# gradslam/gradslam

Measured on AMD Instinct MI355X. Metric: frames/sec PointFusion 640x480 RGB-D, higher is better.
Workload: dtype f32

## Files before the change

### gradslam_amd/csrc/build.py

```python
import os
import subprocess
import sys
from concurrent.futures import ThreadPoolExecutor

HERE = os.path.dirname(os.path.abspath(__file__))
SOURCES = ["gs_frame.hip", "gs_assoc.hip", "gs_fuse.hip", "gs_knn.hip", "gs_icp.hip", "gs_icp_loop.hip", "gs_icp_bwd.hip", "gs_ingest.hip", "gs_render.hip", "gs_prune.hip", "gs_bilateral.hip"]
HEADERS = ["gs_common.h", "gs_env.h", "gs_compact.h", "gs_assoc_dev.h", "gs_knn.h", "gs_knn_bbox.h", "gs_icp_math.h", "gs_icp_persist.h", "gs_icp_timeline.h", os.path.join("..", "..", "include", "gradslam_hip.h")]
LIB = os.path.join(HERE, "libgradslam_hip.so")
FLAGS = ["--offload-arch=gfx950", "-O3", "-std=c++17", "-fPIC", "-ffp-contract=off", "-fno-fast-math", "-fno-slp-vectorize",
         "-fvisibility=hidden", "-Wall", "-Wno-unused-function"]


FLAGS += os.environ.get("GRADSLAM_HIP_BUILD_FLAGS", "").split()


def _hipcc():
    for c in (os.environ.get("HIPCC"), "/opt/rocm/bin/hipcc", "hipcc"):
        if c and (os.path.sep not in c or os.path.exists(c)):
            return c
    raise RuntimeError("hipcc not found")


def _stale(target, deps):
    if not os.path.exists(target):
        return True
    t = os.path.getmtime(target)
    return any(os.path.getmtime(d) > t for d in deps)


def build(force=False, verbose=False):
    hipcc = _hipcc()
    stamp = os.path.join(HERE, ".build_flags")
    flags_now = " ".join(FLAGS)
    if not os.path.exists(stamp) or open(stamp).read() != flags_now:
        force = True
    hdrs = [os.path.join(HERE, h) for h in HEADERS]
    jobs = []
    for s in SOURCES:
        src = os.path.join(HERE, s)
        obj = os.path.join(HERE, s.replace(".hip", ".o"))
        if force or _stale(obj, [src] + hdrs):
            jobs.append([hipcc] + FLAGS + ["-c", src, "-o", obj])

    def run(cmd):
        if verbose:
            print(" ".join(cmd))
        r = subprocess.run(cmd, capture_output=True, text=True)
        if r.returncode != 0:
            raise RuntimeError("hipcc failed:\n%s\n%s" % (" ".join(cmd), r.stderr))
        return r.stderr

    with ThreadPoolExecutor(max_workers=4) as ex:
        for err in ex.map(run, jobs):
            if err.strip() and verbose:
                print(err)
    objs = [os.path.join(HERE, s.replace(".hip", ".o")) for s in SOURCES]
    if force or jobs or _stale(LIB, objs):
        run([hipcc, "--offload-arch=gfx950", "-shared", "-fPIC", "-o", LIB] + objs)
    with open(stamp, "w") as f:
        f.write(flags_now)
    return LIB


if __name__ == "__main__":
    print(build(force="--force" in sys.argv, verbose=True))
```

### gradslam_amd/csrc/gs_common.h

```cpp
#pragma once
#include <hip/hip_runtime.h>
#include <atomic>
#include <stdint.h>
#include <stdio.h>

#include "../../include/gradslam_hip.h"

#define GS_ABI_VERSION 3

constexpr int GS_MAX_BATCH = 8;
struct GsClearJob {
  int n;
  size_t bytes;
  char* ptr[GS_MAX_BATCH];
};
constexpr int GS_CLEAR_ITEMS = 8;
struct GsPixelTables {
  int n;
  uint64_t* key_pix[GS_MAX_BATCH];
  int32_t* best_pix[GS_MAX_BATCH];
  int32_t* any_flag[GS_MAX_BATCH];
  int32_t* call_flag;
};
int gs_frame_maps_batch_clear(const float* depth, int64_t depth_stride_seq, int64_t depth_stride_frame, const float* K16,
                              int n_frames, int frames_per_K, int H, int W, float two_sigma_sq, float* vertex,
                              float* normal, float* alpha, const GsClearJob* job, void* stream,
                              const GsPixelTables* tables = nullptr);

int gs_update_map_fusion_batch_impl(const gs_update_seq* seqs_host, int B, int H, int W, float dist_th, float dot_th,
                                    int renorm_all, void* stream, bool tables_ready);
int32_t* gs_update_map_call_flag(void* scratch_of_first_sequence);
void gs_update_map_tables(void* scratch, int32_t** any_flag, uint64_t** key_pix);

void gs_set_error(const char* fmt, ...);

#define GS_REQUIRE(cond, msg)                  \
  do {                                         \
    if (!(cond)) {                             \
      gs_set_error("%s: %s", __func__, msg);   \
      return GS_ERR_INVALID;                   \
    }                                          \
  } while (0)

#define GS_HIP(call)                                                            \
  do {                                                                          \
    hipError_t e_ = (call);                                                     \
    if (e_ != hipSuccess) {                                                     \
      gs_set_error("%s: %s -> %s", __func__, #call, hipGetErrorString(e_));     \
      return GS_ERR_HIP;                                                        \
    }                                                                           \
  } while (0)

#define GS_LAUNCH_CHECK() GS_HIP(hipGetLastError())

static inline hipStream_t gs_stream(void* s) { return reinterpret_cast<hipStream_t>(s); }
static inline int64_t gs_ceil_div(int64_t a, int64_t b) { return (a + b - 1) / b; }
static inline size_t gs_align(size_t x, size_t a = 256) { return (x + a - 1) / a * a; }

enum GsProfKind { GS_PROF_KNN = 0, GS_PROF_LINEARIZE = 1, GS_PROF_FRAME = 2, GS_PROF_PROJECT = 3,
                  GS_PROF_ASSOC = 4, GS_PROF_FUSE = 5, GS_PROF_COMPACT = 6, GS_PROF_SOLVE = 7, GS_PROF_ICP_FUSED = 8,
                  GS_PROF_KINDS = 9 };
extern std::atomic<bool> g_gs_prof_on;
int gs_prof_open(int kind, double work, hipStream_t st, int launches);
void gs_prof_close(int slot, hipStream_t st);
struct GsProf {
  int slot;
  hipStream_t st;
  GsProf(int kind, double work, hipStream_t s, int launches = 1) : slot(-1), st(s) {
    if (g_gs_prof_on) slot = gs_prof_open(kind, work, s, launches);
  }
  ~GsProf() {
    if (slot >= 0) gs_prof_close(slot, st);
  }
};

#define GS_DEV __device__ __forceinline__

GS_DEV float gs_fma(float a, float b, float c) { return __builtin_fmaf(a, b, c); }

GS_DEV float gs_dot3_fma(float a0, float a1, float a2, float b0, float b1, float b2) {
  float acc = a0 * b0;
  acc = gs_fma(a1, b1, acc);
  acc = gs_fma(a2, b2, acc);
  return acc;
}
GS_DEV float gs_dot3_plain(float a0, float a1, float a2, float b0, float b1, float b2) {
  float p0 = a0 * b0, p1 = a1 * b1, p2 = a2 * b2;
  float s = p0 + p1;
  return s + p2;
}
GS_DEV float gs_norm3(float x, float y, float z) {
  float acc = x * x;
  acc = gs_fma(y, y, acc);
  acc = gs_fma(z, z, acc);
  return __builtin_sqrtf(acc);
}

GS_DEV float gs_expf_spec(float x) {
  if (x < -87.0f) return 0.0f;
  if (x > 88.0f) return __builtin_inff();
  float n = __builtin_rintf(x * 1.44269504088896341f);
  float r = gs_fma(-n, 0.693359375f, x);
  r = gs_fma(-n, -2.12194440e-4f, r);
  float p = 1.9875691500e-4f;
  p = gs_fma(p, r, 1.3981999507e-3f);
  p = gs_fma(p, r, 8.3334519073e-3f);
  p = gs_fma(p, r, 4.1665795894e-2f);
  p = gs_fma(p, r, 1.6666665459e-1f);
  p = gs_fma(p, r, 5.0000001201e-1f);
  float r2 = r * r;
  float y = gs_fma(p, r2, r);
  y = y + 1.0f;
  int32_t bits = __float_as_int(y) + (((int32_t)n) << 23);
// ... 88 lines not shown
```

### gradslam_amd/csrc/gs_env.h

```cpp
#pragma once
#include <stdlib.h>
#include <string.h>

struct GsEnv {
  bool icp_lists;
  int icp_lists_from;
  bool icp_wide;
  bool icp_far;
  bool icp_binned_normals;
  float icp_weak_room;
  bool icp_persist;
  bool icp_lanes_set;
  int icp_lanes;
  int icp_blocks_per_cu;
  const char* icp_timeline;
  const char* icp_persist_timeline;
  bool icp_timeline_it_set; int icp_timeline_it;
  int timeline_it(int numiters) const { return icp_timeline_it_set ? icp_timeline_it : numiters - 1; }
  bool knn_brute;
  int knn_spt;
  bool debug_grid;
};

inline const GsEnv& gs_env() {
  static const GsEnv env = [] {
    const auto num = [](const char* name, int unset) { const char* e = getenv(name); return e ? atoi(e) : unset; };
    GsEnv v;
    v.icp_lists = num("GRADSLAM_HIP_ICP_LISTS", 1) != 0;
    v.icp_lists_from = num("GRADSLAM_HIP_ICP_LISTS_FROM", -1);
    v.icp_wide = num("GRADSLAM_HIP_ICP_WIDE", 1) != 0;
    v.icp_far = num("GRADSLAM_HIP_ICP_FAR", 0) != 0;
    v.icp_binned_normals = num("GRADSLAM_HIP_ICP_BINNED_NORMALS", 1) != 0;
    const char* room = getenv("GRADSLAM_HIP_ICP_WEAK_ROOM");
    v.icp_weak_room = room ? (float)atof(room) : 0.0f;
    if (!(v.icp_weak_room >= 0.0f && v.icp_weak_room < 1.0f)) v.icp_weak_room = 0.0f;
    v.icp_persist = num("GRADSLAM_HIP_ICP_PERSIST", 0) == 1;
    v.icp_lanes_set = getenv("GRADSLAM_HIP_ICP_LANES") != nullptr;
    v.icp_lanes = num("GRADSLAM_HIP_ICP_LANES", 0);
    v.icp_blocks_per_cu = num("GRADSLAM_HIP_ICP_BLOCKS_PER_CU", 0);
    v.icp_timeline = getenv("GRADSLAM_HIP_ICP_TIMELINE");
    v.icp_persist_timeline = getenv("GRADSLAM_HIP_ICP_PERSIST_TIMELINE");
    v.icp_timeline_it_set = getenv("GRADSLAM_HIP_ICP_TIMELINE_IT") != nullptr;
    v.icp_timeline_it = num("GRADSLAM_HIP_ICP_TIMELINE_IT", 0);
    const char* knn = getenv("GRADSLAM_HIP_KNN");
    v.knn_brute = knn && strcmp(knn, "brute") == 0;
    v.knn_spt = num("GRADSLAM_HIP_KNN_SPT", 0);
    v.debug_grid = getenv("GRADSLAM_HIP_DEBUG_GRID") != nullptr;
    return v;
  }();
  return env;
}
```

### gradslam_amd/csrc/gs_frame.hip

```cpp
#include <stdarg.h>
#include <string.h>

#include "gs_compact.h"

static thread_local char g_err[512] = "";

void gs_set_error(const char* fmt, ...) {
  va_list ap;
  va_start(ap, fmt);
  vsnprintf(g_err, sizeof(g_err), fmt, ap);
  va_end(ap);
}

#include <mutex>
#include <vector>
std::atomic<bool> g_gs_prof_on{false};
namespace {
std::mutex g_prof_mu;
struct ProfRec { hipEvent_t a, b; int kind; double work; bool closed; int launches; };
std::vector<ProfRec> g_prof;
size_t g_prof_used = 0;
double g_prof_ms[GS_PROF_KINDS], g_prof_work[GS_PROF_KINDS];
int64_t g_prof_n[GS_PROF_KINDS];
}

int gs_prof_open(int kind, double work, hipStream_t st, int launches) {
  std::lock_guard<std::mutex> lock(g_prof_mu);
  if (!g_gs_prof_on.load() || g_prof_used >= g_prof.size()) return -1;
  ProfRec& r = g_prof[g_prof_used];
  r.kind = kind; r.work = work; r.closed = false; r.launches = launches;
  if (hipEventRecord(r.a, st) != hipSuccess) return -1;
  return (int)g_prof_used++;
}
void gs_prof_close(int slot, hipStream_t st) {
  std::lock_guard<std::mutex> lock(g_prof_mu);
  if ((size_t)slot < g_prof_used && hipEventRecord(g_prof[slot].b, st) == hipSuccess) g_prof[slot].closed = true;
}

extern "C" int gs_profile_begin(int max_records) {
  GS_REQUIRE(max_records > 0 && max_records <= (1 << 20), "max_records out of range");
  std::lock_guard<std::mutex> lock(g_prof_mu);
  while (g_prof.size() < (size_t)max_records) {
    ProfRec r;
    GS_HIP(hipEventCreate(&r.a));
    GS_HIP(hipEventCreate(&r.b));
    r.kind = 0; r.work = 0; r.closed = false; r.launches = 1;
    g_prof.push_back(r);
  }
  g_prof_used = 0;
  for (int k = 0; k < GS_PROF_KINDS; ++k) { g_prof_ms[k] = 0; g_prof_work[k] = 0; g_prof_n[k] = 0; }
  g_gs_prof_on = true;
  return GS_OK;
}
extern "C" int gs_profile_end(void) {
  g_gs_prof_on = false;
  GS_HIP(hipDeviceSynchronize());
  std::lock_guard<std::mutex> lock(g_prof_mu);
  for (size_t i = 0; i < g_prof_used; ++i) {
    const ProfRec& r = g_prof[i];
    if (!r.closed) continue;
    float ms = 0.f;
    if (hipEventElapsedTime(&ms, r.a, r.b) != hipSuccess) continue;
    g_prof_ms[r.kind] += ms; g_prof_work[r.kind] += r.work; g_prof_n[r.kind] += r.launches;
  }
  return GS_OK;
}
extern "C" int gs_profile_read(int kind, double* ms_total, int64_t* launches, double* work_total) {
  GS_REQUIRE(kind >= 0 && kind < GS_PROF_KINDS && ms_total && launches && work_total, "bad arguments");
  std::lock_guard<std::mutex> lock(g_prof_mu);
  *ms_total = g_prof_ms[kind]; *launches = g_prof_n[kind]; *work_total = g_prof_work[kind];
  return GS_OK;
}

extern "C" int gs_abi_version(void) { return GS_ABI_VERSION; }
extern "C" const char* gs_last_error(void) { return g_err; }

extern "C" int64_t gs_scratch_bytes(int64_t n_map, int64_t n_pix) {
  int64_t n = n_map > n_pix ? n_map : n_pix;
  return (int64_t)(gs_cp_scratch_bytes(n) + gs_align(8 * (size_t)(n_pix > 0 ? n_pix : 1)) +
                   gs_align(8 * (size_t)(n_map > 0 ? n_map : 1)) + 4096);
}

__global__ void gs_cp_scan_tiles_kernel(const int32_t* __restrict__ tile_counts, int64_t ntiles,
                                        int64_t* __restrict__ tile_offsets,
                                        int64_t* __restrict__ count_out, GsCount base_count) {
  __shared__ int smem[1024 / GS_WAVE + 1];
  __shared__ int64_t carry;
  if (threadIdx.x == 0) carry = 0;
  __syncthreads();
  for (int64_t t0 = 0; t0 < ntiles; t0 += 1024) {
    int64_t t = t0 + threadIdx.x;
    int c = (t < ntiles) ? tile_counts[t] : 0;
    int total;
    int excl = gs_block_excl_scan<1024>(c, smem, &total);
    if (t < ntiles) tile_offsets[t] = carry + excl;
    __syncthreads();
    if (threadIdx.x == 0) carry += total;
    __syncthreads();
  }
  if (threadIdx.x == 0 && count_out) count_out[0] = gs_count(base_count) + carry;
}

constexpr int FM_TW = 64;
constexpr int FM_TH = 8;
constexpr int FM_LW = FM_TW + 2;
constexpr int FM_LH = FM_TH + 2;

GS_DEV void fm_vertex(float d, int h, int w, const GsKinv& k, float& x, float& y, float& z) {
  float u = (float)w, v = (float)h;
  float ax = k.k00 * u;
  ax = gs_fma(0.0f, v, ax);
  ax = gs_fma(k.k02, 1.0f, ax);
  float ay = 0.0f * u;
  ay = gs_fma(k.k11, v, ay);
  ay = gs_fma(k.k12, 1.0f, ay);
  float az = 0.0f * u;
  az = gs_fma(0.0f, v, az);
  az = gs_fma(1.0f, 1.0f, az);
  float validf = d > 0.0f ? 1.0f : 0.0f;
  x = (ax * d) * validf;
  y = (ay * d) * validf;
  z = (az * d) * validf;
}

struct GsRow3 {
  float x, y, z;
};
GS_DEV void frame_maps_body(const float* __restrict__ depth, const float* __restrict__ K16, int H, int W,
                            float two_sigma_sq, float* __restrict__ vertex, float* __restrict__ normal,
                            float* __restrict__ alpha, uint8_t* __restrict__ valid,
                            uint64_t* __restrict__ key_pix = nullptr, int32_t* __restrict__ best_pix = nullptr) {
  __shared__ float tile[FM_LH][FM_LW];
  const int w_base = blockIdx.x * FM_TW, h_base = blockIdx.y * FM_TH;
  for (int i = threadIdx.x; i < FM_LH * FM_LW; i += 256) {
    int lh = i / FM_LW, lw = i - lh * FM_LW;
    int gh = h_base + lh - 1, gw = w_base + lw - 1;
    gh = gh < 0 ? 0 : (gh > H - 1 ? H - 1 : gh);
    gw = gw < 0 ? 0 : (gw > W - 1 ? W - 1 : gw);
    tile[lh][lw] = depth[(size_t)gh * W + gw];
  }
  __syncthreads();
  const GsKinv k = gs_kinv(K16);
  const int lane = threadIdx.x & 63, wave = threadIdx.x >> 6;
  const int w = w_base + lane;
  if (w >= W) return;
#pragma unroll
  for (int r = 0; r < 2; ++r) {
    const int lh = wave * 2 + r;
    const int h = h_base + lh;
    if (h >= H) continue;
    const size_t p = (size_t)h * W + w;
    const float d = tile[lh + 1][lane + 1];
    float vx, vy, vz;
    fm_vertex(d, h, w, k, vx, vy, vz);
    if (vertex) reinterpret_cast<GsRow3*>(vertex)[p] = GsRow3{vx, vy, vz};
    if (valid) valid[p] = d > 0.0f ? 1 : 0;
    if (alpha) alpha[p] = gs_alpha_of(vx, vy, vz, two_sigma_sq, 1e-7f);
    if (key_pix) { key_pix[p] = ~0ull; best_pix[p] = -1; }
    if (normal) {
      const int w0 = (w < W - 1) ? w : W - 2;
      const int h0 = (h < H - 1) ? h : H - 2;
      const int lw0 = w0 - w_base + 1, lh0 = h0 - h_base + 1;
      float a0x, a0y, a0z, a1x, a1y, a1z, b0x, b0y, b0z, b1x, b1y, b1z;
      fm_vertex(tile[lh + 1][lw0], h, w0, k, a0x, a0y, a0z);
      fm_vertex(tile[lh + 1][lw0 + 1], h, w0 + 1, k, a1x, a1y, a1z);
      fm_vertex(tile[lh0][lane + 1], h0, w, k, b0x, b0y, b0z);
      fm_vertex(tile[lh0 + 1][lane + 1], h0 + 1, w, k, b1x, b1y, b1z);
      const float dhx = a1x - a0x, dhy = a1y - a0y, dhz = a1z - a0z;
      const float dvx = b1x - b0x, dvy = b1y - b0y, dvz = b1z - b0z;
      const float nx = gs_fma(dhy, dvz, -(dhz * dvy));
      const float ny = gs_fma(dhz, dvx, -(dhx * dvz));
      const float nz = gs_fma(dhx, dvy, -(dhy * dvx));
      const float nrm = gs_norm3(nx, ny, nz);
      const float den = (nrm == 0.0f) ? 1.0f : nrm;
      const float validf = d > 0.0f ? 1.0f : 0.0f;
      reinterpret_cast<GsRow3*>(normal)[p] = GsRow3{(nx / den) * validf, (ny / den) * validf, (nz / den) * validf};
    }
  }
}

__global__ void __launch_bounds__(256) gs_frame_maps_kernel(
    const float* __restrict__ depth, const float* __restrict__ K16, int H, int W, float two_sigma_sq,
    float* __restrict__ vertex, float* __restrict__ normal, float* __restrict__ alpha,
    uint8_t* __restrict__ valid) {
  frame_maps_body(depth, K16, H, W, two_sigma_sq, vertex, normal, alpha, valid);
}
__global__ void __launch_bounds__(256) gs_frame_maps_batch_kernel(
    const float* __restrict__ depth, int64_t stride_seq, int64_t stride_frame, const float* __restrict__ K16,
    int frames_per_K, int H, int W, float two_sigma_sq, float* __restrict__ vertex, float* __restrict__ normal,
    float* __restrict__ alpha, const int n_frames, const GsClearJob job, const GsPixelTables tabs) {
  if ((int)blockIdx.z >= n_frames) {
    const size_t blk = ((size_t)(blockIdx.z - n_frames) * gridDim.y + blockIdx.y) * gridDim.x + blockIdx.x;
    const size_t n16 = job.bytes / 16, per = (n16 + 256 * GS_CLEAR_ITEMS - 1) / (256 * GS_CLEAR_ITEMS);
    const size_t r = blk / per;
    if (r >= (size_t)job.n) return;
    float4* dst = reinterpret_cast<float4*>(job.ptr[r]);
    const size_t base = (blk % per) * 256 * GS_CLEAR_ITEMS + threadIdx.x;
#pragma unroll
    for (int u = 0; u < GS_CLEAR_ITEMS; ++u) {
      const size_t i = base + (size_t)u * 256;
      if (i < n16) dst[i] = make_float4(0.0f, 0.0f, 0.0f, 0.0f);
    }
    return;
  }
  const size_t f = blockIdx.z, P = (size_t)H * W;
  const size_t b = f / frames_per_K, l = f % frames_per_K;
  const bool tb = (int)f < tabs.n;
  if (tb && blockIdx.x == 0 && blockIdx.y == 0 && threadIdx.x == 0) {
    tabs.any_flag[f][0] = 0;
    tabs.any_flag[f][1] = 0;
    if (f == 0 && tabs.call_flag) *tabs.call_flag = 0;
  }
  frame_maps_body(depth + b * stride_seq + l * stride_frame, K16 + 16 * b, H, W, two_sigma_sq, vertex + 3 * f * P,
                  normal ? normal + 3 * f * P : nullptr, alpha ? alpha + f * P : nullptr, nullptr,
                  tb ? tabs.key_pix[f] : nullptr, tb ? tabs.best_pix[f] : nullptr);
}

extern "C" int gs_frame_maps_f32(const float* depth, const float* K16, int H, int W,
                                 float two_sigma_sq, float* vertex, float* normal, float* alpha,
                                 uint8_t* valid, void* stream) {
  GS_REQUIRE(depth && K16, "depth and K16 must not be NULL");
  GS_REQUIRE(H >= 2 && W >= 2, "image must be at least 2x2");
  dim3 grid((unsigned)gs_ceil_div(W, FM_TW), (unsigned)gs_ceil_div(H, FM_TH));
  const double bytes = (double)H * W * (4.0 + (vertex ? 12 : 0) + (normal ? 12 : 0) + (alpha ? 4 : 0) + (valid ? 1 : 0));
  GsProf prof(GS_PROF_FRAME, bytes, gs_stream(stream));
  hipLaunchKernelGGL(gs_frame_maps_kernel, grid, dim3(256), 0, gs_stream(stream), depth, K16, H, W,
                     two_sigma_sq, vertex, normal, alpha, valid);
  GS_LAUNCH_CHECK();
  return GS_OK;
}

int gs_frame_maps_batch_clear(const float* depth, int64_t depth_stride_seq, int64_t depth_stride_frame, const float* K16,
                              int n_frames, int frames_per_K, int H, int W, float two_sigma_sq, float* vertex,
                              float* normal, float* alpha, const GsClearJob* job, void* stream,
                              const GsPixelTables* tables) {
  GS_REQUIRE(depth && K16 && vertex, "depth, K16 and vertex must not be NULL");
  GsPixelTables tabs;
  tabs.n = 0; tabs.call_flag = nullptr;
  if (tables && tables->n > 0) {
    GS_REQUIRE(tables->n <= GS_MAX_BATCH && tables->n <= n_frames, "bad pixel tables");
    tabs = *tables;
  }
  GS_REQUIRE(H >= 2 && W >= 2, "image must be at least 2x2");
  GS_REQUIRE(n_frames > 0 && n_frames <= 65535 && frames_per_K > 0 && n_frames % frames_per_K == 0, "bad frame count");
  GS_REQUIRE(depth_stride_frame >= (int64_t)H * W && depth_stride_seq >= 0, "bad depth strides");
  dim3 grid((unsigned)gs_ceil_div(W, FM_TW), (unsigned)gs_ceil_div(H, FM_TH), (unsigned)n_frames);
  GsClearJob none;
  none.n = 0; none.bytes = 0;
  if (job && job->n > 0 && job->bytes > 0) {
    GS_REQUIRE(job->n <= GS_MAX_BATCH && job->bytes % 16 == 0, "bad clear job");
    const int64_t per = gs_ceil_div((int64_t)(job->bytes / 16), 256 * GS_CLEAR_ITEMS);
    const int64_t slices = gs_ceil_div(per * job->n, (int64_t)grid.x * grid.y);
    GS_REQUIRE(n_frames + slices <= 65535, "clear job too large for the launch");
    grid.z += (unsigned)slices;
  } else {
    job = &none;
  }
  const double bytes = (double)n_frames * H * W * (4.0 + 12.0 + (normal ? 12 : 0) + (alpha ? 4 : 0)) +
                       (double)tabs.n * H * W * 12.0;
  GsProf prof(GS_PROF_FRAME, bytes, gs_stream(stream));
  hipLaunchKernelGGL(gs_frame_maps_batch_kernel, grid, dim3(256), 0, gs_stream(stream), depth, depth_stride_seq,
                     depth_stride_frame, K16, frames_per_K, H, W, two_sigma_sq, vertex, normal, alpha, n_frames, *job, tabs);
  GS_LAUNCH_CHECK();
  return GS_OK;
}

extern "C" int gs_frame_maps_batch_f32(const float* depth, int64_t depth_stride_seq, int64_t depth_stride_frame,
                                       const float* K16, int n_frames, int frames_per_K, int H, int W,
                                       float two_sigma_sq, float* vertex, float* normal, float* alpha, void* stream) {
  return gs_frame_maps_batch_clear(depth, depth_stride_seq, depth_stride_frame, K16, n_frames, frames_per_K, H, W,
                                   two_sigma_sq, vertex, normal, alpha, nullptr, stream);
}

__global__ void __launch_bounds__(256) gs_global_maps_kernel(
    const float* __restrict__ vertex, const float* __restrict__ normal,
    const float* __restrict__ depth, const float* __restrict__ pose16, int64_t P,
    float* __restrict__ gvertex, float* __restrict__ gnormal) {
  const int64_t p = (int64_t)blockIdx.x * 256 + threadIdx.x;
  if (p >= P) return;
  float T[12];
#pragma unroll
  for (int i = 0; i < 12; ++i) T[i] = pose16[i];
  if (gvertex) {
    const float v0 = vertex[3 * p], v1 = vertex[3 * p + 1], v2 = vertex[3 * p + 2];
    const float validf = depth[p] > 0.0f ? 1.0f : 0.0f;
    float g0, g1, g2;
    gs_rigid_fma(T, v0, v1, v2, g0, g1, g2);
    gvertex[3 * p] = g0 * validf;
    gvertex[3 * p + 1] = g1 * validf;
    gvertex[3 * p + 2] = g2 * validf;
  }
  if (gnormal) {
    const float n0 = normal[3 * p], n1 = normal[3 * p + 1], n2 = normal[3 * p + 2];
    gnormal[3 * p] = gs_dot3_fma(T[0], T[1], T[2], n0, n1, n2);
    gnormal[3 * p + 1] = gs_dot3_fma(T[4], T[5], T[6], n0, n1, n2);
    gnormal[3 * p + 2] = gs_dot3_fma(T[8], T[9], T[10], n0, n1, n2);
  }
}

extern "C" int gs_global_maps_f32(const float* vertex, const float* normal, const float* depth,
                                  const float* pose16, int H, int W, float* gvertex,
                                  float* gnormal, void* stream) {
  GS_REQUIRE(H > 0 && W > 0, "empty image");
  GS_REQUIRE(!gvertex || (vertex && depth), "gvertex needs vertex and depth");
  GS_REQUIRE(!gnormal || normal, "gnormal needs normal");
  const int64_t P = (int64_t)H * W;
  hipStream_t st = gs_stream(stream);
  if (!pose16) {
    if (gvertex) GS_HIP(hipMemcpyAsync(gvertex, vertex, P * 12, hipMemcpyDeviceToDevice, st));
    if (gnormal) GS_HIP(hipMemcpyAsync(gnormal, normal, P * 12, hipMemcpyDeviceToDevice, st));
    return GS_OK;
  }
  GsProf prof(GS_PROF_FRAME, (double)P * (4.0 + (gvertex ? 24 : 0) + (gnormal ? 24 : 0)), st);
  hipLaunchKernelGGL(gs_global_maps_kernel, dim3((unsigned)gs_ceil_div(P, 256)), dim3(256), 0, st,
                     vertex, normal, depth, pose16, P, gvertex, gnormal);
  GS_LAUNCH_CHECK();
  return GS_OK;
}

__global__ void __launch_bounds__(256) gs_alpha_kernel(const float* __restrict__ pts, int64_t n,
                                                       float two_sigma_sq, float eps,
                                                       float* __restrict__ alpha) {
  const int64_t i = (int64_t)blockIdx.x * 256 + threadIdx.x;
  if (i >= n) return;
  alpha[i] = gs_alpha_of(pts[3 * i], pts[3 * i + 1], pts[3 * i + 2], two_sigma_sq, eps);
}

extern "C" int gs_alpha_f32(const float* points, int64_t n, float two_sigma_sq, float eps,
                            float* alpha, void* stream) {
  GS_REQUIRE(n >= 0, "negative n");
  if (n == 0) return GS_OK;
  GS_REQUIRE(points && alpha, "NULL pointer");
  hipLaunchKernelGGL(gs_alpha_kernel, dim3((unsigned)gs_ceil_div(n, 256)), dim3(256), 0,
                     gs_stream(stream), points, n, two_sigma_sq, eps, alpha);
  GS_LAUNCH_CHECK();
  return GS_OK;
}

__global__ void __launch_bounds__(256) gs_alpha_bwd_kernel(const float* __restrict__ pts, int64_t n, float two_sigma_sq,
                                                           float eps, const float* __restrict__ alpha_bar,
                                                           float* __restrict__ pts_bar, float* __restrict__ sigma_terms) {
  const int64_t i = (int64_t)blockIdx.x * 256 + threadIdx.x;
  if (i >= n) return;
  const float x = pts[3 * i], y = pts[3 * i + 1], z = pts[3 * i + 2];
  float S = x * x + y * y;
// ... 226 lines not shown
```

### gradslam_amd/csrc/gs_fuse.hip

```cpp
#include "gs_assoc_dev.h"
#include "gs_compact.h"

__global__ void __launch_bounds__(256) gs_fuse_init_kernel(int32_t* __restrict__ pix_of, int64_t n,
                                                           int32_t* __restrict__ any_flag) {
  const int64_t i = (int64_t)blockIdx.x * 256 + threadIdx.x;
  if (i == 0) *any_flag = 0;
  if (i < n) pix_of[i] = -1;
}

__global__ void __launch_bounds__(256) gs_fuse_scatter_kernel(const int32_t* __restrict__ best_pix,
                                                              int64_t P, GsCount n_map_c,
                                                              int32_t* __restrict__ pix_of,
                                                              int32_t* __restrict__ any_flag) {
  const int64_t p = (int64_t)blockIdx.x * 256 + threadIdx.x;
  if (p >= P) return;
  const int32_t n = best_pix[p];
  if (n >= 0 && n < gs_count(n_map_c)) {
    pix_of[n] = (int32_t)p;
    *any_flag = 1;
  }
}

struct FrameGlobalMaps {
  const float* __restrict__ gvertex;
  const float* __restrict__ gnormal;
  __device__ void operator()(const int64_t p, float* fp, float* fn) const {
#pragma unroll
    for (int k = 0; k < 3; ++k) {
      fp[k] = gvertex[3 * p + k];
      fn[k] = gnormal[3 * p + k];
    }
  }
  __device__ void vertex_of(const int64_t p, float* fp) const {
#pragma unroll
    for (int k = 0; k < 3; ++k) fp[k] = gvertex[3 * p + k];
  }
  __device__ void normal_of(const int64_t p, float* fn) const {
#pragma unroll
    for (int k = 0; k < 3; ++k) fn[k] = gnormal[3 * p + k];
  }
};
struct FrameLocalMaps {
  const float* __restrict__ vertex;
  const float* __restrict__ normal;
  float T[12];
  __device__ void operator()(const int64_t p, float* fp, float* fn) const {
    float v[3], n[3];
#pragma unroll
    for (int k = 0; k < 3; ++k) {
      v[k] = vertex[3 * p + k];
      n[k] = normal[3 * p + k];
    }
    const float validf = v[2] > 0.0f ? 1.0f : 0.0f;
    float g0, g1, g2;
    gs_rigid_fma(T, v[0], v[1], v[2], g0, g1, g2);
    fp[0] = g0 * validf; fp[1] = g1 * validf; fp[2] = g2 * validf;
    fn[0] = gs_dot3_fma(T[0], T[1], T[2], n[0], n[1], n[2]);
    fn[1] = gs_dot3_fma(T[4], T[5], T[6], n[0], n[1], n[2]);
    fn[2] = gs_dot3_fma(T[8], T[9], T[10], n[0], n[1], n[2]);
  }
  __device__ void vertex_of(const int64_t p, float* fp) const {
    float v[3];
#pragma unroll
    for (int k = 0; k < 3; ++k) v[k] = vertex[3 * p + k];
    const float validf = v[2] > 0.0f ? 1.0f : 0.0f;
    float g0, g1, g2;
    gs_rigid_fma(T, v[0], v[1], v[2], g0, g1, g2);
    fp[0] = g0 * validf; fp[1] = g1 * validf; fp[2] = g2 * validf;
  }
  __device__ void normal_of(const int64_t p, float* fn) const {
    float n[3];
#pragma unroll
    for (int k = 0; k < 3; ++k) n[k] = normal[3 * p + k];
    fn[0] = gs_dot3_fma(T[0], T[1], T[2], n[0], n[1], n[2]);
    fn[1] = gs_dot3_fma(T[4], T[5], T[6], n[0], n[1], n[2]);
    fn[2] = gs_dot3_fma(T[8], T[9], T[10], n[0], n[1], n[2]);
  }
};
GS_DEV FrameLocalMaps frame_local_maps(const float* vertex, const float* normal, const float* pose16) {
  FrameLocalMaps f;
  f.vertex = vertex; f.normal = normal;
#pragma unroll
  for (int i = 0; i < 12; ++i) f.T[i] = pose16[i];
  return f;
}

template <bool HAVE_VERTEX = false, class Frame>
GS_DEV void fuse_merge_row(float* __restrict__ points, float* __restrict__ normals, float* __restrict__ colors,
                           float* __restrict__ ccounts, const int64_t n, const int32_t p, const Frame& frame,
                           const float* __restrict__ rgb, const float* __restrict__ alpha, const float cc,
                           const float* fv = nullptr) {
  const float a = p >= 0 ? alpha[p] : 0.0f;
  float P[3], N[3], C[3], fp[3] = {0.0f, 0.0f, 0.0f}, fn[3] = {0.0f, 0.0f, 0.0f}, fc[3] = {0.0f, 0.0f, 0.0f};
#pragma unroll
  for (int k = 0; k < 3; ++k) {
    P[k] = points[3 * n + k];
    N[k] = normals[3 * n + k];
    C[k] = colors[3 * n + k];
  }
  if (p >= 0) {
    if (HAVE_VERTEX) {
      frame.normal_of((int64_t)p, fn);
#pragma unroll
      for (int k = 0; k < 3; ++k) fp[k] = fv[k];
    } else {
      frame((int64_t)p, fp, fn);
    }
#pragma unroll
    for (int k = 0; k < 3; ++k) fc[k] = rgb[3 * (int64_t)p + k];
  }
  const float cc2 = cc + a;
  const float inv = 1.0f / (cc2 == 0.0f ? 1.0f : cc2);
#pragma unroll
  for (int k = 0; k < 3; ++k) {
    P[k] = ((cc * P[k]) + (a * fp[k])) * inv;
    N[k] = ((cc * N[k]) + (a * fn[k])) * inv;
    C[k] = ((cc * C[k]) + (a * fc[k])) * inv;
  }
#pragma unroll
  for (int k = 0; k < 3; ++k) points[3 * n + k] = P[k];
#pragma unroll
  for (int k = 0; k < 3; ++k) normals[3 * n + k] = N[k];
#pragma unroll
  for (int k = 0; k < 3; ++k) colors[3 * n + k] = C[k];
  ccounts[n] = cc2;
}

__global__ void __launch_bounds__(256) gs_fuse_merge_kernel(
    float* __restrict__ points, float* __restrict__ normals, float* __restrict__ colors,
    float* __restrict__ ccounts, GsCount n_map_c, const int32_t* __restrict__ pix_of,
    const int32_t* __restrict__ any_flag, const float* __restrict__ gvertex,
    const float* __restrict__ gnormal, const float* __restrict__ rgb, const float* __restrict__ alpha,
    int renorm_all) {
  const int64_t n = (int64_t)blockIdx.x * 256 + threadIdx.x;
  if (n >= gs_count(n_map_c)) return;
  if (*any_flag == 0 && renorm_all != 2) return;
  const int32_t p = pix_of[n];
  if (p < 0 && !renorm_all) return;
  fuse_merge_row(points, normals, colors, ccounts, n, p, FrameGlobalMaps{gvertex, gnormal}, rgb, alpha, ccounts[n]);
}

struct PredNewPixel {
  const float* depth;
  const int32_t* best_pix;
  __device__ bool operator()(int64_t p) const {
    return depth[p] > 0.0f && (best_pix == nullptr || best_pix[p] < 0);
  }
};
template <class Frame>
struct EmitAppendT {
  float* points;
  float* normals;
  float* colors;
  float* ccounts;
  GsCount n_map;
  Frame frame;
  const float* rgb;
  const float* alpha;
  __device__ void operator()(int64_t p, int64_t pos) const {
    const int64_t r = gs_count(n_map) + pos;
    float v[3], nn[3] = {0.0f, 0.0f, 0.0f}, c[3] = {0.0f, 0.0f, 0.0f};
    frame.vertex_of(p, v);
    if (normals) frame.normal_of(p, nn);
    if (colors) {
#pragma unroll
      for (int k = 0; k < 3; ++k) c[k] = rgb[3 * p + k];
    }
    const float a = ccounts ? alpha[p] : 0.0f;
#pragma unroll
    for (int k = 0; k < 3; ++k) points[3 * r + k] = v[k];
    if (normals) {
#pragma unroll
      for (int k = 0; k < 3; ++k) normals[3 * r + k] = nn[k];
    }
    if (colors) {
#pragma unroll
      for (int k = 0; k < 3; ++k) colors[3 * r + k] = c[k];
    }
    if (ccounts) ccounts[r] = a;
  }
};
typedef EmitAppendT<FrameGlobalMaps> EmitAppend;

static int fuse_append(float* points, float* normals, float* colors, float* ccounts, GsCount n_map_c,
                       int64_t capacity, const int32_t* best_pix, const float* gvertex, const float* gnormal,
                       const float* rgb, const float* alpha, const float* depth, int H, int W, int renorm_all,
                       int64_t* new_count_out, void* scratch, void* stream) {
  const int64_t n_map_host = n_map_c.host;
  GS_REQUIRE(H > 0 && W > 0 && n_map_host >= 0 && capacity >= n_map_host, "bad sizes");
  GS_REQUIRE(points && normals && colors && ccounts && best_pix && gvertex && gnormal && rgb && alpha &&
                 depth && new_count_out && scratch,
             "NULL pointer");
  hipStream_t st = gs_stream(stream);
  const int64_t P = (int64_t)H * W;
  const int64_t n_map = n_map_host;
  char* base = reinterpret_cast<char*>(scratch) + gs_cp_scratch_bytes(P > n_map ? P : n_map);
  int32_t* any_flag = reinterpret_cast<int32_t*>(base);
  int32_t* pix_of = reinterpret_cast<int32_t*>(base + 256);
  GsProf prof(GS_PROF_FUSE, 88.0 * (double)n_map + 45.0 * (double)P, st);
  if (n_map > 0) {
    hipLaunchKernelGGL(gs_fuse_init_kernel, dim3((unsigned)gs_ceil_div(n_map, 256)), dim3(256), 0, st,
                       pix_of, n_map, any_flag);
    hipLaunchKernelGGL(gs_fuse_scatter_kernel, dim3((unsigned)gs_ceil_div(P, 256)), dim3(256), 0, st,
                       best_pix, P, n_map_c, pix_of, any_flag);
    hipLaunchKernelGGL(gs_fuse_merge_kernel, dim3((unsigned)gs_ceil_div(n_map, 256)), dim3(256), 0, st,
                       points, normals, colors, ccounts, n_map_c, pix_of, any_flag, gvertex, gnormal, rgb,
                       alpha, renorm_all);
    GS_LAUNCH_CHECK();
  }
  EmitAppend emit{points, normals, colors, ccounts, n_map_c, FrameGlobalMaps{gvertex, gnormal}, rgb, alpha};
  return gs_compact(GsCount{P, nullptr}, PredNewPixel{depth, best_pix}, emit, new_count_out, n_map_c, capacity,
                    scratch, st);
}

extern "C" int gs_fuse_append_f32(float* points, float* normals, float* colors, float* ccounts,
                                  int64_t n_map_host, int64_t capacity, const int32_t* best_pix,
                                  const float* gvertex, const float* gnormal, const float* rgb,
                                  const float* alpha, const float* depth, int H, int W, int renorm_all,
                                  int64_t* new_count_out, void* scratch, void* stream) {
  return fuse_append(points, normals, colors, ccounts, GsCount{n_map_host, nullptr}, capacity, best_pix, gvertex,
                     gnormal, rgb, alpha, depth, H, W, renorm_all, new_count_out, scratch, stream);
}
extern "C" int gs_fuse_append_dc_f32(float* points, float* normals, float* colors, float* ccounts,
                                     int64_t n_map_bound, const int64_t* n_map_dev, int64_t capacity,
                                     const int32_t* best_pix, const float* gvertex, const float* gnormal,
                                     const float* rgb, const float* alpha, const float* depth, int H, int W,
                                     int renorm_all, int64_t* new_count_out, void* scratch, void* stream) {
  GS_REQUIRE(n_map_dev && capacity >= n_map_bound + (int64_t)H * W, "device-count fuse needs capacity >= bound + H*W");
  return fuse_append(points, normals, colors, ccounts, GsCount{n_map_bound, n_map_dev}, capacity, best_pix,
                     gvertex, gnormal, rgb, alpha, depth, H, W, renorm_all, new_count_out, scratch, stream);
}

static int append_valid(float* points, float* normals, float* colors, float* ccounts, GsCount n_map_c,
                        int64_t capacity, const float* gvertex, const float* gnormal, const float* rgb,
                        const float* alpha, const float* depth, int H, int W, int64_t* new_count_out,
                        void* scratch, void* stream) {
  GS_REQUIRE(H > 0 && W > 0 && n_map_c.host >= 0 && capacity >= n_map_c.host, "bad sizes");
  GS_REQUIRE(points && gvertex && depth && new_count_out && scratch, "NULL pointer");
  EmitAppend emit{points, gnormal ? normals : nullptr, rgb ? colors : nullptr, alpha ? ccounts : nullptr,
                  n_map_c, FrameGlobalMaps{gvertex, gnormal}, rgb, alpha};
  return gs_compact(GsCount{(int64_t)H * W, nullptr}, PredNewPixel{depth, nullptr}, emit, new_count_out, n_map_c,
                    capacity, scratch, gs_stream(stream));
}
extern "C" int gs_append_valid_f32(float* points, float* normals, float* colors, float* ccounts,
                                   int64_t n_map_host, int64_t capacity, const float* gvertex,
                                   const float* gnormal, const float* rgb, const float* alpha,
                                   const float* depth, int H, int W, int64_t* new_count_out,
                                   void* scratch, void* stream) {
  return append_valid(points, normals, colors, ccounts, GsCount{n_map_host, nullptr}, capacity, gvertex, gnormal,
                      rgb, alpha, depth, H, W, new_count_out, scratch, stream);
}
// ... 63 lines not shown
  const float* P_bar;
  const float* N_bar;
  const float* C_bar;
  const float* F_bar;
  int64_t n_old;
  float* gv_bar;
  float* gn_bar;
  float* rgb_bar;
  float* alpha_bar;
  __device__ void operator()(int64_t p, int64_t pos) const {
    const int64_t r = n_old + pos;
#pragma unroll
    for (int k = 0; k < 3; ++k) {
      gv_bar[3 * p + k] = P_bar[3 * r + k];
      gn_bar[3 * p + k] = N_bar[3 * r + k];
      rgb_bar[3 * p + k] = C_bar[3 * r + k];
    }
    alpha_bar[p] = F_bar[r];
  }
};

extern "C" int gs_fuse_append_backward_f32(const float* points, const float* normals, const float* colors,
                                           const float* ccounts, int64_t n_old, const int32_t* best_pix,
                                           const float* gvertex, const float* gnormal, const float* rgb,
                                           const float* alpha, const float* depth, int H, int W, int renorm_all,
                                           const float* P_bar, const float* N_bar, const float* C_bar,
                                           const float* F_bar, int64_t n_new, float* old_points_bar,
                                           float* old_normals_bar, float* old_colors_bar, float* old_ccounts_bar,
                                           float* gvertex_bar, float* gnormal_bar, float* rgb_bar, float* alpha_bar,
                                           void* scratch, void* stream) {
  GS_REQUIRE(H > 0 && W > 0 && n_old >= 0 && n_new >= n_old, "bad sizes");
  GS_REQUIRE(best_pix && gvertex && gnormal && rgb && alpha && depth && P_bar && N_bar && C_bar && F_bar && gvertex_bar &&
                 gnormal_bar && rgb_bar && alpha_bar && scratch,
             "NULL pointer");
  hipStream_t st = gs_stream(stream);
  const int64_t P = (int64_t)H * W;
  GS_HIP(hipMemsetAsync(gvertex_bar, 0, 12 * (size_t)P, st));
  GS_HIP(hipMemsetAsync(gnormal_bar, 0, 12 * (size_t)P, st));
  GS_HIP(hipMemsetAsync(rgb_bar, 0, 12 * (size_t)P, st));
  GS_HIP(hipMemsetAsync(alpha_bar, 0, 4 * (size_t)P, st));
  char* base = reinterpret_cast<char*>(scratch) + gs_cp_scratch_bytes(P > n_old ? P : n_old);
  int32_t* any_flag = reinterpret_cast<int32_t*>(base);
  int32_t* pix_of = reinterpret_cast<int32_t*>(base + 256);
  if (n_old > 0) {
    GS_REQUIRE(points && normals && colors && ccounts && old_points_bar && old_normals_bar && old_colors_bar &&
                   old_ccounts_bar,
               "NULL pointer");
    const GsCount n_old_c{n_old, nullptr};
    hipLaunchKernelGGL(gs_fuse_init_kernel, dim3((unsigned)gs_ceil_div(n_old, 256)), dim3(256), 0, st, pix_of, n_old,
                       any_flag);
    hipLaunchKernelGGL(gs_fuse_scatter_kernel, dim3((unsigned)gs_ceil_div(P, 256)), dim3(256), 0, st, best_pix, P,
                       n_old_c, pix_of, any_flag);
    hipLaunchKernelGGL(gs_fuse_bwd_rows_kernel, dim3((unsigned)gs_ceil_div(n_old, 256)), dim3(256), 0, st, points,
                       normals, colors, ccounts, n_old, pix_of, any_flag, gvertex, gnormal, rgb, alpha, renorm_all, P_bar,
                       N_bar, C_bar, F_bar, old_points_bar, old_normals_bar, old_colors_bar, old_ccounts_bar,
                       gvertex_bar, gnormal_bar, rgb_bar, alpha_bar);
    GS_LAUNCH_CHECK();
  }
  EmitAppendBackward emit{P_bar, N_bar, C_bar, F_bar, n_old, gvertex_bar, gnormal_bar, rgb_bar, alpha_bar};
  int64_t* cnt = reinterpret_cast<int64_t*>(base + 128);
  return gs_compact(P, PredNewPixel{depth, best_pix}, emit, cnt, 0, n_new - n_old, scratch, st);
}

constexpr int32_t MU_TIE_MARK = 0x7fffffff;
struct MuSeq {
  float* points; float* normals; float* colors; float* ccounts;
  GsCount n_map;
  int64_t capacity;
  const float* vertex; const float* normal; const float* depth; const float* rgb; const float* alpha;
  const float* pose16; const float* K16;
  float* gvertex; float* gnormal;
  int32_t* best_pix;
  int64_t* new_count_out;
  int32_t* any_flag;
  uint64_t* key_pix;
  int32_t* tile_counts;
  int32_t* pix;
  int32_t* pix_of;
};
struct MuBatch {
  int B, H, W, renorm_all;
  int64_t P, ntiles;
  float u_hi, v_hi, dist_th, dot_th;
  int32_t* call_flag;
  int zero_call_flag;
  MuSeq s[GS_MAX_BATCH];
};

__global__ void __launch_bounds__(256) gs_mu_pixel_init_kernel(const MuBatch mb) {
  const MuSeq& q = mb.s[blockIdx.x % mb.B];
  const int64_t p = (int64_t)(blockIdx.x / mb.B) * 256 + threadIdx.x;
  if (p == 0) { q.any_flag[0] = 0; q.any_flag[1] = 0; }
  if (blockIdx.x == 0 && threadIdx.x == 0 && mb.zero_call_flag) *mb.call_flag = 0;
  if (p >= mb.P) return;
  float T[12];
#pragma unroll
  for (int i = 0; i < 12; ++i) T[i] = q.pose16[i];
  const float validf = q.depth[p] > 0.0f ? 1.0f : 0.0f;
  float g0, g1, g2;
  gs_rigid_fma(T, q.vertex[3 * p], q.vertex[3 * p + 1], q.vertex[3 * p + 2], g0, g1, g2);
  q.gvertex[3 * p] = g0 * validf;
  q.gvertex[3 * p + 1] = g1 * validf;
  q.gvertex[3 * p + 2] = g2 * validf;
  const float n0 = q.normal[3 * p], n1 = q.normal[3 * p + 1], n2 = q.normal[3 * p + 2];
  q.gnormal[3 * p] = gs_dot3_fma(T[0], T[1], T[2], n0, n1, n2);
  q.gnormal[3 * p + 1] = gs_dot3_fma(T[4], T[5], T[6], n0, n1, n2);
  q.gnormal[3 * p + 2] = gs_dot3_fma(T[8], T[9], T[10], n0, n1, n2);
  q.key_pix[p] = ~0ull;
  q.best_pix[p] = -1;
}

__global__ void __launch_bounds__(256) gs_mu_project_key_kernel(const MuBatch mb) {
  const MuSeq& q = mb.s[blockIdx.x % mb.B];
  const int64_t n = (int64_t)(blockIdx.x / mb.B) * 256 + threadIdx.x;
  if (n >= gs_count(q.n_map)) return;
  const GsCamera c = gs_camera(q.pose16, q.K16);
  const int32_t p = gs_project_point(c, q.points[3 * n], q.points[3 * n + 1], q.points[3 * n + 2], mb.H, mb.W, mb.u_hi,
                                     mb.v_hi);
  int32_t pk = -1;
  if (p >= 0) {
    float fp[3], fn[3];
    if (q.gvertex) FrameGlobalMaps{q.gvertex, q.gnormal}((int64_t)p, fp, fn);
    else frame_local_maps(q.vertex, q.normal, q.pose16)((int64_t)p, fp, fn);
    if (gs_is_similar_v(q.points, q.normals, fp, fn, n, mb.dist_th, mb.dot_th)) {
      const uint64_t k = gs_assoc_key_v(q.points, q.ccounts, fp, n);
      const unsigned long long old = atomicMin(reinterpret_cast<unsigned long long*>(&q.key_pix[p]), (unsigned long long)k);
      if (old == (unsigned long long)k) {
        q.best_pix[p] = MU_TIE_MARK;
        q.any_flag[1] = 1;
      }
      pk = p;
    }
  }
  q.pix[n] = pk;
}

GS_DEV void mu_settle_ties(const MuSeq& q, const unsigned blk, const unsigned nblk) {
  if (q.any_flag[1] == 0) return;
  const int64_t n_map = gs_count(q.n_map);
  for (int64_t n = (int64_t)blk * GS_CP_BLOCK + threadIdx.x; n < n_map; n += (int64_t)nblk * GS_CP_BLOCK) {
    const int32_t p = q.pix[n];
    if (p < 0 || q.best_pix[p] == -1) continue;
    float fp[3];
    if (q.gvertex) FrameGlobalMaps{q.gvertex, q.gnormal}.vertex_of((int64_t)p, fp);
    else frame_local_maps(q.vertex, q.normal, q.pose16).vertex_of((int64_t)p, fp);
    if (gs_assoc_key_v(q.points, q.ccounts, fp, n) == q.key_pix[p]) atomicMin(reinterpret_cast<unsigned*>(&q.best_pix[p]), (unsigned)n);
  }
}

__global__ void __launch_bounds__(GS_CP_BLOCK) gs_mu_winner_count_kernel(const MuBatch mb) {
  __shared__ int smem[GS_CP_BLOCK / GS_WAVE + 1];
  const MuSeq& q = mb.s[blockIdx.x % mb.B];
  const unsigned blk = blockIdx.x / mb.B;
  const int64_t base = (int64_t)blk * GS_CP_TILE + (int64_t)threadIdx.x * GS_CP_ITEMS;
  int c = 0;
  uint64_t kk[GS_CP_ITEMS];
  float dd[GS_CP_ITEMS];
#pragma unroll
  for (int i = 0; i < GS_CP_ITEMS; ++i) {
    const int64_t pc = base + i < mb.P ? base + i : mb.P - 1;
    kk[i] = q.key_pix[pc];
    dd[i] = q.depth[pc];
  }
  bool any = false;
#pragma unroll
  for (int i = 0; i < GS_CP_ITEMS; ++i) {
    const int64_t p = base + i;
    if (p < mb.P) {
      const bool matched = kk[i] != ~0ull;
      any = any || matched;
      if (dd[i] > 0.0f && !matched) ++c;
    }
  }
  if (any) {
    q.any_flag[0] = 1;
    *mb.call_flag = 1;
  }
  int total;
  (void)gs_block_excl_scan<GS_CP_BLOCK>(c, smem, &total);
  if (threadIdx.x == 0) q.tile_counts[blk] = total;
  mu_settle_ties(q, blk, gridDim.x / mb.B);
}

template <class Frame>
GS_DEV void mu_merge_row(const MuBatch& mb, const MuSeq& q, const int64_t n, const Frame& frame) {
  int32_t p = q.pix[n];
  const float cc = q.ccounts[n];
  float fp[3] = {0.0f, 0.0f, 0.0f};
  if (p >= 0) {
    const uint64_t kp = q.key_pix[p];
    bool win = (uint32_t)(kp >> 32) == gs_assoc_key_hi(cc);
    if (win) {
      frame.vertex_of((int64_t)p, fp);
      const int32_t bp = q.best_pix[p];
      win = (uint32_t)kp == gs_assoc_key_lo_v(q.points, fp, n) && (bp == -1 || bp == (int32_t)n);
      if (win && bp == -1) q.best_pix[p] = (int32_t)n;
    }
    if (!win) p = -1;
  }
  if (p < 0 && !mb.renorm_all) return;
  fuse_merge_row<true>(q.points, q.normals, q.colors, q.ccounts, n, p, frame, q.rgb, q.alpha, cc, fp);
}

GS_DEV void mu_merge_body(const MuBatch& mb, const unsigned bid) {
  const MuSeq& q = mb.s[bid % mb.B];
  const int64_t n = (int64_t)(bid / mb.B) * 256 + threadIdx.x;
  if (n >= gs_count(q.n_map)) return;
  if (*mb.call_flag == 0) return;
  if (q.gvertex) mu_merge_row(mb, q, n, FrameGlobalMaps{q.gvertex, q.gnormal});
  else mu_merge_row(mb, q, n, frame_local_maps(q.vertex, q.normal, q.pose16));
}

GS_DEV void mu_append_body(const MuBatch& mb, const unsigned bid) {
  __shared__ int smem[GS_CP_BLOCK / GS_WAVE + 1];
  const MuSeq& q = mb.s[bid % mb.B];
  const unsigned blk = bid / mb.B;
  int before = 0, all = 0;
  for (int64_t t = threadIdx.x; t < mb.ntiles; t += GS_CP_BLOCK) {
    const int v = q.tile_counts[t];
    all += v;
    if (t < (int64_t)blk) before += v;
  }
  int tile_prefix, total_new, tile_new;
  (void)gs_block_excl_scan<GS_CP_BLOCK>(before, smem, &tile_prefix);
  (void)gs_block_excl_scan<GS_CP_BLOCK>(all, smem, &total_new);
  const int64_t n_map = gs_count(q.n_map);
  if (blk == 0 && threadIdx.x == 0) q.new_count_out[0] = n_map + total_new;
  const int64_t base = (int64_t)blk * GS_CP_TILE + (int64_t)threadIdx.x * GS_CP_ITEMS;
  bool keep[GS_CP_ITEMS];
  int c = 0;
  {
    uint64_t kk[GS_CP_ITEMS];
    float dd[GS_CP_ITEMS];
#pragma unroll
    for (int i = 0; i < GS_CP_ITEMS; ++i) {
      const int64_t pc = base + i < mb.P ? base + i : mb.P - 1;
      kk[i] = q.key_pix[pc];
      dd[i] = q.depth[pc];
    }
#pragma unroll
    for (int i = 0; i < GS_CP_ITEMS; ++i) {
      keep[i] = base + i < mb.P && dd[i] > 0.0f && kk[i] == ~0ull;
      c += keep[i] ? 1 : 0;
    }
  }
  int w = gs_block_excl_scan<GS_CP_BLOCK>(c, smem, &tile_new);
  __shared__ unsigned short loc_s[GS_CP_TILE];
#pragma unroll
  for (int i = 0; i < GS_CP_ITEMS; ++i) {
    if (keep[i]) loc_s[w++] = (unsigned short)(threadIdx.x * GS_CP_ITEMS + i);
  }
  __syncthreads();
  const int64_t tile_base = (int64_t)blk * GS_CP_TILE;
  if (q.gvertex) {
    const EmitAppend emit{q.points, q.normals, q.colors, q.ccounts, q.n_map, FrameGlobalMaps{q.gvertex, q.gnormal}, q.rgb, q.alpha};
    for (int r = threadIdx.x; r < tile_new; r += GS_CP_BLOCK) {
      const int64_t pos = (int64_t)tile_prefix + r;
      if (n_map + pos < q.capacity) emit(tile_base + loc_s[r], pos);
    }
  } else {
    const EmitAppendT<FrameLocalMaps> emit{q.points, q.normals, q.colors, q.ccounts, q.n_map,
                                           frame_local_maps(q.vertex, q.normal, q.pose16), q.rgb, q.alpha};
    for (int r = threadIdx.x; r < tile_new; r += GS_CP_BLOCK) {
      const int64_t pos = (int64_t)tile_prefix + r;
      if (n_map + pos < q.capacity) emit(tile_base + loc_s[r], pos);
    }
  }
}

static_assert(GS_CP_BLOCK == 256, "merge and append blocks share a launch");
__global__ void __launch_bounds__(256) gs_mu_merge_append_kernel(const MuBatch mb, const unsigned nb_append) {
  if (blockIdx.x < nb_append) mu_append_body(mb, blockIdx.x);
  else mu_merge_body(mb, blockIdx.x - nb_append);
}

extern "C" int64_t gs_update_map_scratch_bytes(int64_t n_map_bound, int H, int W) {
  const int64_t P = (int64_t)H * W;
  return (int64_t)(256 + gs_align(8 * (size_t)P) + gs_align(4 * (size_t)gs_cp_tiles(P)) +
                   2 * gs_align(4 * (size_t)(n_map_bound > 0 ? n_map_bound : 1)) + 4096);
}

int32_t* gs_update_map_call_flag(void* scratch0) { return reinterpret_cast<int32_t*>(scratch0) + 32; }
void gs_update_map_tables(void* scratch, int32_t** any_flag, uint64_t** key_pix) {
  *any_flag = reinterpret_cast<int32_t*>(scratch);
  *key_pix = reinterpret_cast<uint64_t*>(reinterpret_cast<char*>(scratch) + 256);
}

static int update_chunk(const gs_update_seq* seqs, int B, int H, int W, float dist_th, float dot_th, int renorm_all,
                        hipStream_t st, int phase, int32_t* call_flag, bool first_chunk, bool tables_ready) {
  MuBatch mb;
  mb.B = B; mb.H = H; mb.W = W; mb.renorm_all = renorm_all;
  mb.call_flag = call_flag; mb.zero_call_flag = first_chunk ? 1 : 0;
  mb.P = (int64_t)H * W;
  mb.ntiles = gs_cp_tiles(mb.P);
  mb.u_hi = (float)((double)W - 0.999); mb.v_hi = (float)((double)H - 0.999);
  mb.dist_th = dist_th; mb.dot_th = dot_th;
  int64_t n_max = 0;
  double bytes_assoc = 0.0, bytes_fuse = 0.0;
  for (int b = 0; b < B; ++b) {
    const gs_update_seq& u = seqs[b];
    const int64_t n_map = u.map.n_bound;
    n_max = n_map > n_max ? n_map : n_max;
    char* q = reinterpret_cast<char*>(u.scratch);
    MuSeq& m = mb.s[b];
    m.points = u.map.points; m.normals = u.map.normals; m.colors = u.map.colors; m.ccounts = u.map.ccounts;
    m.n_map = GsCount{u.map.n_bound, u.map.n_dev};
    m.capacity = u.map.capacity;
    m.vertex = u.vertex; m.normal = u.normal; m.depth = u.depth; m.rgb = u.rgb; m.alpha = u.alpha;
    m.pose16 = u.pose16; m.K16 = u.K16;
    m.gvertex = u.gvertex; m.gnormal = u.gnormal; m.best_pix = u.best_pix; m.new_count_out = u.new_count_out;
    m.any_flag = reinterpret_cast<int32_t*>(q); q += 256;
    m.key_pix = reinterpret_cast<uint64_t*>(q); q += gs_align(8 * (size_t)mb.P);
    m.tile_counts = reinterpret_cast<int32_t*>(q); q += gs_align(4 * (size_t)mb.ntiles);
    m.pix = reinterpret_cast<int32_t*>(q); q += gs_align(4 * (size_t)(n_map > 0 ? n_map : 1));
    m.pix_of = reinterpret_cast<int32_t*>(q);
    bytes_assoc += 64.0 * (double)n_map;
    bytes_fuse += 96.0 * (double)n_map + 49.0 * (double)mb.P;
  }
  const unsigned uB = (unsigned)B;
  const unsigned pb = uB * (unsigned)gs_ceil_div(mb.P, 256), nb = uB * (unsigned)gs_ceil_div(n_max > 0 ? n_max : 1, 256);
  if (phase == 0) {
    if (!tables_ready) {
      GsProf prof(GS_PROF_FRAME, (double)B * (double)mb.P * 64.0, st);
      hipLaunchKernelGGL(gs_mu_pixel_init_kernel, dim3(pb), dim3(256), 0, st, mb);
    }
    if (n_max > 0) {
      GsProf prof(GS_PROF_ASSOC, bytes_assoc, st, 1);
      hipLaunchKernelGGL(gs_mu_project_key_kernel, dim3(nb), dim3(256), 0, st, mb);
    }
    GsProf prof(GS_PROF_FUSE, bytes_fuse / 3.0, st, 1);
    hipLaunchKernelGGL(gs_mu_winner_count_kernel, dim3(uB * (unsigned)mb.ntiles), dim3(GS_CP_BLOCK), 0, st, mb);
  } else {
    GsProf prof(GS_PROF_FUSE, bytes_fuse * (2.0 / 3.0), st, 1);
    const unsigned nb_append = uB * (unsigned)mb.ntiles;
    hipLaunchKernelGGL(gs_mu_merge_append_kernel, dim3(nb_append + (n_max > 0 ? nb : 0u)), dim3(256), 0, st, mb, nb_append);
  }
  GS_LAUNCH_CHECK();
  return GS_OK;
}

int gs_update_map_fusion_batch_impl(const gs_update_seq* seqs_host, int B, int H, int W, float dist_th, float dot_th,
                                    int renorm_all, void* stream, bool tables_ready) {
  GS_REQUIRE(seqs_host && B > 0 && H > 0 && W > 0, "bad arguments");
  GS_REQUIRE((int64_t)H * W < (1ll << 31), "too large for int32 indices");
  for (int b = 0; b < B; ++b) {
    const gs_update_seq& u = seqs_host[b];
    GS_REQUIRE(u.map.n_bound >= 0 && u.map.n_bound < 0x7fffffff, "bad map size");
    GS_REQUIRE(u.map.capacity >= u.map.n_bound + (int64_t)H * W, "capacity must cover n_bound + H*W rows");
    GS_REQUIRE(u.map.points && u.map.normals && u.map.colors && u.map.ccounts && u.vertex && u.normal && u.depth && u.rgb &&
                   u.alpha && u.pose16 && u.K16 && u.best_pix && u.new_count_out && u.scratch,
               "NULL pointer");
    GS_REQUIRE((u.gvertex && u.gnormal) || (tables_ready && !u.gvertex && !u.gnormal), "gvertex / gnormal: both or none");
    GS_REQUIRE(u.new_count_out != u.map.n_dev, "new_count_out must not alias the map's device count");
  }
  hipStream_t st = gs_stream(stream);
  int32_t* call_flag = gs_update_map_call_flag(seqs_host[0].scratch);
  for (int phase = 0; phase < 2; ++phase) {
    for (int c0 = 0; c0 < B; c0 += GS_MAX_BATCH) {
      const int nb = B - c0 < GS_MAX_BATCH ? B - c0 : GS_MAX_BATCH;
      const int rc = update_chunk(seqs_host + c0, nb, H, W, dist_th, dot_th, renorm_all, st, phase, call_flag, c0 == 0,
                                  tables_ready);
      if (rc != GS_OK) return rc;
    }
  }
  return GS_OK;
}

extern "C" int gs_update_map_fusion_batch_f32(const gs_update_seq* seqs_host, int B, int H, int W, float dist_th,
                                              float dot_th, int renorm_all, void* stream) {
  return gs_update_map_fusion_batch_impl(seqs_host, B, H, W, dist_th, dot_th, renorm_all, stream, false);
}

extern "C" int gs_update_map_fusion_dc_f32(float* points, float* normals, float* colors, float* ccounts,
                                           int64_t n_map_bound, const int64_t* n_map_dev, int64_t capacity,
                                           const float* vertex, const float* normal, const float* depth,
                                           const float* rgb, const float* alpha, const float* pose16,
                                           const float* K16, int H, int W, float dist_th, float dot_th,
                                           int renorm_all, float* gvertex, float* gnormal, int32_t* best_pix,
                                           int64_t* new_count_out, void* scratch, void* stream) {
  gs_update_seq u;
  u.map = gs_map_view{points, normals, colors, ccounts, capacity, n_map_bound, n_map_dev};
  u.vertex = vertex; u.normal = normal; u.depth = depth; u.rgb = rgb; u.alpha = alpha;
  u.pose16 = pose16; u.K16 = K16;
  u.gvertex = gvertex; u.gnormal = gnormal; u.best_pix = best_pix; u.new_count_out = new_count_out; u.scratch = scratch;
  return gs_update_map_fusion_batch_f32(&u, 1, H, W, dist_th, dot_th, renorm_all, stream);
}
```

### gradslam_amd/csrc/gs_icp_loop.hip

```cpp
#include <stdlib.h>
#include <string.h>

#include <memory>
#include <mutex>
#include <optional>
#include <type_traits>

#include "gs_env.h"
#include "gs_icp_math.h"
#include "gs_knn.h"
#include "gs_knn_bbox.h"

constexpr int GS_ICP_MAX_ITERS = 1024;
struct GsIcpState {
  IcpSmall s[2];
  float trace[GS_ICP_MAX_ITERS * 12];
};

struct TapePtrs {
  float* src;
  int32_t* idx;
  float* sys;
};
GS_DEV void tape_write_sys(float* __restrict__ sys, int it, const double* S, float damp) {
// ... 933 lines not shown
  IcpSmall sm;
  for (int i = 0; i < 16; ++i) {
    sm.T_total[i] = init16[i];
    sm.T_step[i] = init16[i];
    sm.Tr[i] = (i % 5 == 0) ? 1.0f : 0.0f;
  }
  for (int i = 0; i < 8; ++i) sm.xi[i] = 0.0f;
  sm.damp = damp;
  sm.err = 0.0f;
  sm.pad[0] = sm.pad[1] = 0.0f;
  return sm;
}
__global__ void gs_icp_init_kernel(GsIcpState* __restrict__ st, const float* __restrict__ init16, float damp,
                                   int numiters, const float* __restrict__ compose16, float* __restrict__ out_T16) {
  if (threadIdx.x != 0) return;
  const IcpSmall sm = icp_state_init(init16, damp);
  st->s[0] = sm;
  st->s[1] = sm;
  if (numiters == 0) icp_write_result(sm, compose16, out_T16);
}

template <class T>
static T* gs_at(void* base, size_t offset) { return reinterpret_cast<T*>(reinterpret_cast<char*>(base) + offset); }
struct GsTake { size_t end = 0; size_t operator()(size_t n) { end += n; return end - n; } };

constexpr int ICP_ROWRED_DOUBLES = 32;
struct IcpLayout { size_t state, rowred, sync, best, srcA, srcB, partials[2], grid, total; };
static IcpLayout icp_layout(int64_t n_src, int64_t n_tgt) {
  GsTake take;
  IcpLayout L;
  L.state = take(gs_align(sizeof(GsIcpState)));
  L.rowred = take(gs_align(sizeof(double) * ICP_ROWRED_DOUBLES));
  L.sync = L.rowred + sizeof(double) * LIN_NV;
  static_assert(8 * ICP_ROWRED_DOUBLES >= 8 * LIN_NV + 4 * PS_WORDS, "the sync record does not fit behind rowred + LIN_NV");
  L.best = take(gs_align(8 * (size_t)n_src));
  L.srcA = take(gs_align(12 * (size_t)n_src)); L.srcB = take(gs_align(12 * (size_t)n_src));
  for (int k = 0; k < 2; ++k) L.partials[k] = take(gs_align(sizeof(double) * LIN_NV * icp_rows(n_src)));
  L.grid = take(gs_knn_grid_scratch_bytes(n_src, n_tgt));
  L.total = take.end + 4096;
  return L;
}
struct IcpScratch {
  GsIcpState* state;
  double* rowred;
  unsigned* sync;
  unsigned long long* best; float *srcA, *srcB;
  double* partials[2]; void* grid;
};
static IcpScratch icp_carve(void* p, const IcpLayout& L) {
  return IcpScratch{gs_at<GsIcpState>(p, L.state), gs_at<double>(p, L.rowred), gs_at<unsigned>(p, L.sync),
                    gs_at<unsigned long long>(p, L.best), gs_at<float>(p, L.srcA), gs_at<float>(p, L.srcB),
                    {gs_at<double>(p, L.partials[0]), gs_at<double>(p, L.partials[1])}, gs_at<void>(p, L.grid)};
}

extern "C" int64_t gs_icp_scratch_bytes(int64_t n_src, int64_t n_tgt) { return (int64_t)icp_layout(n_src < 1 ? 1 : n_src, n_tgt).total; }

static int icp_tape_finish(void* tape, const GsIcpState* state, int64_t n_src, int numiters, hipStream_t st) {
  GsIcpTape t = gs_icp_tape_carve(tape, n_src, numiters);
  if (numiters > 0)
    GS_HIP(hipMemcpyAsync(t.trace, state->trace, sizeof(float) * 12 * (size_t)numiters, hipMemcpyDeviceToDevice, st));
  return GS_OK;
}

static double icp_alg_bytes(int numiters, int64_t n_slots, int64_t n_queries, int64_t n_binned) {
  const double rows = (double)gs_ceil_div(n_slots, FS_QPB);
  const double full = 12.0 * n_slots + 36.0 * n_queries + 8.0 * LIN_NV * rows + 16.0 * n_binned;
  const double look = 12.0 * n_slots + 24.0 * n_queries + 8.0 * rows + 16.0 * n_binned;
  return (double)numiters * (full + look);
}

struct LocSeq {
  const float* vertex;
  const float* depth;
  const float* pose16;
  float* lattice;
  GsIcpState* state;
  float* out_pose16;
  char* clear_ptr;
  int64_t* n_valid;
  int* far_n;
  int* lstat;
  float4* wl_cq;
  unsigned* sync;
};
struct LocBatch {
  int B, W, ds, Wl;
  int64_t n_lat;
  size_t clear_bytes;
  float damp;
  int numiters;
  int count_valid;
  LocSeq s[GS_MAX_BATCH];
};
constexpr int LP_CLEAR_ITEMS = 8;

GS_DEV void loc_prep_block(const LocBatch& lb, const unsigned bid, const unsigned nb_lat) {
  const LocSeq& q = lb.s[bid % lb.B];
  const unsigned blk = bid / lb.B;
  if (blk < nb_lat) {
    const int64_t e = (int64_t)blk * 256 + threadIdx.x;
    int valid = 0;
    if (e < lb.n_lat) {
      const int64_t p = (e / lb.Wl) * lb.ds * (int64_t)lb.W + (e % lb.Wl) * lb.ds;
      float g0 = __builtin_nanf(""), g1 = g0, g2 = g0;
      if (q.depth[p] > 0.0f) {
        float T[12];
#pragma unroll
        for (int i = 0; i < 12; ++i) T[i] = q.pose16[i];
        gs_rigid_fma(T, q.vertex[3 * p], q.vertex[3 * p + 1], q.vertex[3 * p + 2], g0, g1, g2);
        valid = 1;
      }
      q.lattice[3 * e] = g0; q.lattice[3 * e + 1] = g1; q.lattice[3 * e + 2] = g2;
      if (q.wl_cq) q.wl_cq[e] = make_float4(0.0f, 0.0f, 0.0f, 0.0f);
    }
    const unsigned long long m = lb.count_valid ? __ballot(valid) : 0ull;
    if ((threadIdx.x & 63) == 0 && m) atomicAdd(reinterpret_cast<unsigned long long*>(q.n_valid), (unsigned long long)__popcll(m));
    if (blk == 0 && threadIdx.x == 0) {
      float id[16];
      for (int i = 0; i < 16; ++i) id[i] = (i % 5 == 0) ? 1.0f : 0.0f;
      const IcpSmall sm = icp_state_init(id, lb.damp);
      q.state->s[0] = sm;
      q.state->s[1] = sm;
      if (q.far_n)
        for (int i = 0; i < FS_FAR_PASSES; ++i) q.far_n[i] = 0;
      if (q.lstat)
        for (int i = 0; i < 3 * GL_STAT_LAUNCHES; ++i) q.lstat[i] = 0;
      if (q.sync)
        for (int i = 0; i < PS_WORDS; ++i) q.sync[i] = 0u;
      if (lb.numiters == 0) icp_write_result(sm, q.pose16, q.out_pose16);
    }
    return;
  }
  float4* dst = reinterpret_cast<float4*>(q.clear_ptr);
  const size_t n16 = lb.clear_bytes / 16;
  const size_t base = (size_t)(blk - nb_lat) * 256 * LP_CLEAR_ITEMS + threadIdx.x;
#pragma unroll
  for (int u = 0; u < LP_CLEAR_ITEMS; ++u) {
    const size_t i = base + (size_t)u * 256;
    if (i < n16) dst[i] = make_float4(0.0f, 0.0f, 0.0f, 0.0f);
  }
}
__global__ void __launch_bounds__(256) gs_loc_prep_kernel(const LocBatch lb, unsigned nb_lat) {
  loc_prep_block(lb, blockIdx.x, nb_lat);
}
static_assert(GB_BLOCK == 256, "lattice and bbox blocks share a launch");
__global__ void __launch_bounds__(256) gs_loc_prep_bbox_kernel(const LocBatch lb, const GsGridBatch gb, const unsigned nb_lat,
                                                               const float u_hi, const float v_hi) {
  const unsigned n_prep = (unsigned)lb.B * nb_lat;
  if (blockIdx.x < n_prep) loc_prep_block(lb, blockIdx.x, nb_lat);
  else gridb_bbox_block(gb, blockIdx.x - n_prep, u_hi, v_hi);
}

static int64_t loc_lattice(int H, int W, int ds) { return (int64_t)((H + ds - 1) / ds) * ((W + ds - 1) / ds); }

struct ListMem {
  float4* lq;
  uint32_t* ls;
  int* stat;
};

struct FarMem {
  uint32_t* c;
  float4* cq;
  int* idx;
  int* n;
};

struct FarBuildSeq {
  const float* src;
  const int* idx;
  const int* n;
  const GsGrid* gp;
  const int* cell_start;
  const float4* sorted;
  float* d2prev;
  FarMem m;
};
struct FarBuildBatch {
  int B;
  FarBuildSeq s[GS_MAX_BATCH];
};
constexpr int FAR_BLOCK = 512;
constexpr int FAR_BLOCKS_PER_SEQ = 64;
__global__ void __launch_bounds__(FAR_BLOCK) gs_icp_far_build_kernel(const FarBuildBatch fb) {
  const FarBuildSeq& q = fb.s[blockIdx.x % fb.B];
  const int blk = (int)(blockIdx.x / fb.B);
  const int n = *q.n;
  if (blk >= n) return;
  constexpr int NG = FAR_BLOCK / FS_HG;
  __shared__ float qs[NG][3];
  __shared__ float d1_s[NG];
  __shared__ uint8_t flag_s[NG];
// ... 78 lines not shown
}

struct LocCarve {
  float* lattice; int64_t* n_valid;
  IcpScratch sc; GridMem gm; ListMem lm;
  FarMem fm; int* far_out4;
};
static LocCarve loc_carve(void* p, const LocLayout& L) {
  const IcpScratch sc = icp_carve(gs_at<char>(p, L.icp), L.sc);
  return LocCarve{gs_at<float>(p, L.lattice), gs_at<int64_t>(p, L.n_valid), sc,
                  grid_carve(sc.grid, L.n_lat, L.rows),
                  ListMem{gs_at<float4>(p, L.lq), gs_at<uint32_t>(p, L.ls), gs_at<int>(p, L.lstat)},
                  FarMem{gs_at<uint32_t>(p, L.far_c), gs_at<float4>(p, L.far_cq), gs_at<int>(p, L.far_idx), gs_at<int>(p, L.far_n)},
                  gs_at<int>(p, L.far_out4)};
}
static LocCarve loc_carve_of(const void* scratch, int H, int W, int ds, int64_t map_rows) {
  return loc_carve(const_cast<void*>(scratch), loc_layout(loc_lattice(H, W, ds), map_rows));
}

struct IcpEnginePlan {
  bool far_on, wide_on, lists_on, persist_on;
  bool binned_normals;
  bool reduce_rows;
  int lists_from;
  IcpHalfPlan half;
  int ps_it0, ps_nb, ps_upb;
  float weak_room;
  int lmode(int it, bool look_ahead) const {
    if (!lists_on || it < lists_from) return 0;
    if (it > lists_from) return 2;
    return look_ahead ? (persist_on ? 3 : 1) : 0;
  }
};
static IcpEnginePlan icp_engine_plan(const GsEnv& env, const IcpDevice& dev, int B, int64_t n_lat, int numiters,
                                     const LocLayout* layouts) {
  IcpEnginePlan p;
  const int64_t rows = (int64_t)icp_rows(n_lat);
  p.binned_normals = env.icp_binned_normals; p.weak_room = env.icp_weak_room;
  p.lists_from = env.icp_lists_from >= 0 ? env.icp_lists_from : FS_LISTS_FROM;
  p.reduce_rows = rows > FS_REDUCE_ROWS;
  p.far_on = env.icp_far && numiters > 0;
  p.wide_on = env.icp_wide && !p.far_on && numiters > 0;
  p.ps_upb = (int)gs_ceil_div(rows, PS_CUS_PER_XCD);
  p.ps_nb = (int)gs_ceil_div(rows, p.ps_upb > 0 ? p.ps_upb : 1);
  const bool persist_asked = env.icp_persist && env.icp_lists && !p.far_on && B <= (int)GS_XCDS && p.ps_upb <= PS_UPB &&
                             numiters > p.lists_from + 1 && !env.icp_timeline && !env.icp_lanes_set && dev.ps_fits &&
                             p.binned_normals;
  p.half = icp_half_plan(env, dev.cus, n_lat, B, p.far_on ? 4 : (persist_asked ? 2 : 8));
  p.lists_on = env.icp_lists && !p.far_on && p.half.upb * p.half.G * FS_QPB <= FS_BLOCK;
  for (int b = 0; b < B && p.lists_on; ++b) p.lists_on = loc_lists_fit(layouts[b]);
  p.persist_on = persist_asked && p.half.G == 2 && p.lists_on;
  p.ps_it0 = p.persist_on ? p.lists_from + 1 : numiters;
  return p;
}
static IcpEnginePlan icp_plain_plan(const IcpHalfPlan& half, int64_t n_src, int numiters) {
  IcpEnginePlan p{};
  p.binned_normals = true; p.reduce_rows = icp_rows(n_src) > FS_REDUCE_ROWS;
  p.half = half; p.ps_it0 = numiters;
  return p;
}

struct IcpSolveView {
  const float* src0;
  const float *tgt, *tn; GsCount n_tgt;
  IcpScratch sc; GridMem gm;
  int64_t* out_idx;
  TapePtrs tape;
  IcpHalfLists lists; IcpHalfWide wide; FarMem far;
  const float* compose16; float* out_T16;
  unsigned* sync;
};

static void loc_bind(const gs_localize_seq* seqs, int B, int H, int W, int ds, const gs_icp_params* prm,
                     const IcpEnginePlan& plan, LocCarve* c, LocBatch& lb, GsGridBatch& gb, IcpSolveView* v) {
  lb.B = gb.B = B; lb.W = gb.W = W; gb.H = H; lb.ds = gb.ds = ds;
  gb.listed = 1;
  lb.Wl = (W + ds - 1) / ds; lb.n_lat = loc_lattice(H, W, ds); lb.damp = prm->damp; lb.numiters = prm->numiters;
  gb.cells_cap = gs_knn_grid_cells_cap(lb.n_lat);
  for (int b = 0; b < B; ++b) {
    const gs_localize_seq& q = seqs[b];
    if (!plan.binned_normals) c[b].gm.sorted_n = nullptr;
    lb.s[b] = LocSeq{q.vertex, q.depth, q.prev_pose16, c[b].lattice, c[b].sc.state, q.out_pose16,
                     reinterpret_cast<char*>(c[b].gm.g), c[b].n_valid, c[b].fm.n, c[b].lm.stat,
                     plan.wide_on ? c[b].fm.cq : nullptr, c[b].sc.sync};
    gb.s[b] = GsGridSeq{q.map.points, GsCount{q.map.n_bound, q.map.n_dev}, nullptr, q.prev_pose16, q.K16,
                        plan.binned_normals ? q.map.normals : nullptr, c[b].gm};
    v[b] = IcpSolveView{c[b].lattice, q.map.points, q.map.normals, GsCount{q.map.n_bound, q.map.n_dev}, c[b].sc, c[b].gm,
                        nullptr, TapePtrs{nullptr, nullptr, nullptr},
                        plan.lists_on ? IcpHalfLists{c[b].lm.lq, c[b].lm.ls, c[b].lm.stat, c[b].sc.sync + PS_WEAK}
                                      : IcpHalfLists{nullptr, nullptr, nullptr, nullptr},
                        plan.wide_on ? IcpHalfWide{c[b].fm.cq, c[b].fm.c} : IcpHalfWide{nullptr, nullptr},
                        plan.far_on ? c[b].fm : FarMem{nullptr, nullptr, nullptr, nullptr},
                        q.prev_pose16, q.out_pose16, plan.persist_on ? c[b].sc.sync : nullptr};
  }
  lb.count_valid = g_gs_prof_on ? 1 : 0;
  lb.clear_bytes = gs_knn_grid_clear_bytes(c[0].gm, gb.cells_cap);
}

static int loc_prep(const gs_localize_seq* seqs, const LocBatch& lb, const GsGridBatch& gb, hipStream_t st, bool grid_cleared) {
  const int B = lb.B;
  if (g_gs_prof_on)
    for (int b = 0; b < B; ++b) GS_HIP(hipMemsetAsync(lb.s[b].n_valid, 0, 8, st));
  const unsigned nb_lat = (unsigned)gs_ceil_div(lb.n_lat, 256);
  const unsigned nb_clear = (unsigned)gs_ceil_div((int64_t)(lb.clear_bytes / 16), 256 * LP_CLEAR_ITEMS);
  double bytes = 0.0;
  for (int b = 0; b < B; ++b) bytes += 28.0 * lb.n_lat + 12.0 * seqs[b].map.n_bound + 16.0 * gb.cells_cap;
  GsProf prof(GS_PROF_COMPACT, bytes, st, grid_cleared ? 4 : 5);
  if (grid_cleared) {
    const float u_hi = (float)((double)gb.W - 0.999), v_hi = (float)((double)gb.H - 0.999);
    hipLaunchKernelGGL(gs_loc_prep_bbox_kernel, dim3((unsigned)B * nb_lat + gs_knn_gridb_bbox_blocks(gb)), dim3(256), 0, st,
                       lb, gb, nb_lat, u_hi, v_hi);
    return gs_knn_grid_build_batch(gb, st, true);
  }
  hipLaunchKernelGGL(gs_loc_prep_kernel, dim3((unsigned)B * (nb_lat + nb_clear)), dim3(256), 0, st, lb, nb_lat);
  return gs_knn_grid_build_batch(gb, st);
}

static int loc_prof_bytes(int B, const LocCarve* c, int64_t n_lat, int numiters, hipStream_t st, double* bytes) {
  for (int b = 0; b < B; ++b) {
    unsigned hits = 0; int64_t nv = 0;
    GS_HIP(hipMemcpyAsync(&hits, c[b].gm.bbox + 6, 4, hipMemcpyDeviceToHost, st));
    GS_HIP(hipMemcpyAsync(&nv, c[b].n_valid, 8, hipMemcpyDeviceToHost, st));
    GS_HIP(hipStreamSynchronize(st));
    *bytes += icp_alg_bytes(numiters, n_lat, nv, hits);
  }
  return GS_OK;
}

static const char* icp_params_error(const gs_icp_params* prm) {
  if (!(prm->numiters >= 0 && prm->numiters <= GS_ICP_MAX_ITERS)) return "numiters must be in [0, 1024]";
  return prm->mode == 0 || prm->mode == 1 ? nullptr : "mode must be 0 (ICP) or 1 (gradICP)";
}

struct IcpHalfIo { const double* rows_in; double* rows_out; const IcpSmall* st_in; IcpSmall* st_out; };
static IcpHalfIo icp_half_io(const IcpScratch& sc, int h) {
  return IcpHalfIo{sc.partials[(h + 1) & 1], sc.partials[h & 1], &sc.state->s[h & 1], &sc.state->s[(h + 1) & 1]};
}
static float* icp_cloud(const IcpSolveView& v, int it, int64_t n_src) {
  return v.tape.src ? v.tape.src + (size_t)it * 3 * (size_t)n_src : ((it & 1) ? v.sc.srcB : v.sc.srcA);
}
static int32_t* icp_tape_idx(const IcpSolveView& v, int it, int look_ahead, int64_t n_src) {
  return v.tape.idx ? v.tape.idx + ((size_t)it * 2 + look_ahead) * (size_t)n_src : nullptr;
}

static void loc_half_iterations(const IcpSolveView* v, int B, const IcpEnginePlan& plan, GsCount n_src_c,
                                const gs_icp_params* prm, hipStream_t st, bool prof_rows) {
  const int64_t n_src = n_src_c.host;
  IcpHalfBatch hb;
  hb.B = B; hb.weak_room = plan.weak_room;
  for (int b = 0; b < B; ++b) { hb.w[b] = v[b].wide; hb.l[b] = v[b].lists; }
  for (int it = 0; it < plan.ps_it0; ++it) {
    int h = 2 * it;
    for (int b = 0; b < B; ++b) {
      const IcpSolveView& q = v[b];
      const IcpHalfIo io = icp_half_io(q.sc, h);
      hb.s[b] = IcpHalfSeq{it == 0 ? q.src0 : icp_cloud(q, it - 1, n_src), icp_cloud(q, it, n_src), q.tgt, q.tn, q.n_tgt, q.gm.g,
                           q.gm.cell_start, q.gm.sorted, q.gm.sorted_n, reinterpret_cast<float*>(q.sc.best),
                           io.rows_in, io.rows_out, io.st_in, io.st_out, q.sc.state->trace, q.out_idx,
                           icp_tape_idx(q, it, 0, n_src), nullptr, q.far.cq, q.far.c, q.far.idx, q.far.n};
    }
    icp_half_launch<true>(plan.half, hb, n_src_c, prm, it, 0, st, plan.lmode(it, false));
    if (plan.far_on && fs_far_pass(it) >= 0) {
      const int fp = fs_far_pass(it);
      FarBuildBatch fbb; fbb.B = B;
      for (int b = 0; b < B; ++b)
        fbb.s[b] = FarBuildSeq{icp_cloud(v[b], it, n_src), v[b].far.idx + (int64_t)fp * n_src, v[b].far.n + fp,
                               v[b].gm.g, v[b].gm.cell_start, v[b].gm.sorted, reinterpret_cast<float*>(v[b].sc.best), v[b].far};
      hipLaunchKernelGGL(gs_icp_far_build_kernel, dim3((unsigned)B * FAR_BLOCKS_PER_SEQ), dim3(FAR_BLOCK), 0, st, fbb);
    }
    ++h;
    if (plan.reduce_rows) {
      std::optional<GsProf> prof;
      if (prof_rows) prof.emplace(GS_PROF_SOLVE, 1.0, st);
      IcpRowsBatch rb; rb.B = B;
      for (int b = 0; b < B; ++b) { rb.in[b] = icp_half_io(v[b].sc, h).rows_in; rb.out[b] = v[b].sc.rowred; }
      hipLaunchKernelGGL(gs_icp_reduce_rows_batch_kernel, dim3((unsigned)B), dim3(FS_BLOCK), 0, st, rb, n_src_c);
    }
    for (int b = 0; b < B; ++b) {
      const IcpSolveView& q = v[b];
      const IcpHalfIo io = icp_half_io(q.sc, h);
      IcpHalfSeq& u = hb.s[b];
      u.src_in = icp_cloud(q, it, n_src); u.src_out = nullptr;
      u.partials_in = plan.reduce_rows ? q.sc.rowred : io.rows_in; u.partials_out = io.rows_out;
      u.st_in = io.st_in; u.st_out = io.st_out;
      u.out_idx = nullptr; u.tape_idx = icp_tape_idx(q, it, 1, n_src); u.tape_sys = q.tape.sys;
    }
    icp_half_launch<false>(plan.half, hb, n_src_c, prm, it, plan.reduce_rows ? 1 : 0, st, plan.lmode(it, true));
  }
}

static void loc_persist(const IcpSolveView* v, int B, const IcpEnginePlan& plan, int64_t n_lat, const gs_icp_params* prm,
                        hipStream_t st) {
  IcpPersistBatch pb;
  pb.B = B; pb.nb = plan.ps_nb; pb.upb = plan.ps_upb; pb.h0 = 2 * plan.ps_it0; pb.tl_h = 0; pb.timeline = nullptr;
  for (int b = 0; b < B; ++b) {
// ... 60 lines not shown
    if (g_gs_prof_on) {
      int64_t n_binned = n_tgt;
      if (flt.listed) {
        unsigned hits = 0;
        GS_HIP(hipMemcpyAsync(&hits, v.gm.bbox + 6, 4, hipMemcpyDeviceToHost, st));
        GS_HIP(hipStreamSynchronize(st));
        n_binned = hits;
      }
      prof_bytes = icp_alg_bytes(prm->numiters, n_src, n_src, n_binned);
    }
    const IcpEnginePlan plan = icp_plain_plan(icp_half_plan(gs_env(), icp_device().cus, n_src, 1), n_src, prm->numiters);
    {
      GsProf prof(GS_PROF_ICP_FUSED, prof_bytes, st, 2 * prm->numiters);
      loc_half_iterations(&v, 1, plan, n_src_c, prm, st, true);
    }
    loc_finish(&v, 1, plan, n_src_c, prm, st);
    GS_LAUNCH_CHECK();
    if (tape) return icp_tape_finish(tape, sc.state, n_src, prm->numiters, st);
    return GS_OK;
  }

  GS_HIP(hipMemsetAsync(sc.best, 0xff, 8 * (size_t)n_src, st));
  const int nblk = (int)gs_ceil_div(n_src, LIN_BLOCK);
  double* partials = sc.partials[0];
  const float* cur_in = src;
  for (int it = 0; it < prm->numiters; ++it) {
    float* cur = cloud(it);
    gs_knn_brute_launch(cur_in, sc.state->s[0].T_step, cur, n_src, tgt, n_tgt, sc.best, st);
    {
      GsProf prof(GS_PROF_LINEARIZE, 44.0 * (double)n_src, st);
      hipLaunchKernelGGL((gs_icp_linearize_kernel<true>), dim3(nblk), dim3(LIN_BLOCK), 0, st, cur, nullptr, n_src,
                         tgt, tgt_normals, n_tgt, sc.best, prm->dist_thresh, partials, out_idx, tidx(it, 0));
    }
    {
      GsProf prof(GS_PROF_SOLVE, 1.0, st);
      hipLaunchKernelGGL(gs_icp_solve_kernel, dim3(1), dim3(SUM_BLOCK), 0, st, partials, nblk, sc.state, it, tp.sys);
    }
    gs_knn_brute_launch(cur, sc.state->s[0].Tr, nullptr, n_src, tgt, n_tgt, sc.best, st);
    {
      GsProf prof(GS_PROF_LINEARIZE, 44.0 * (double)n_src, st);
      hipLaunchKernelGGL((gs_icp_linearize_kernel<false>), dim3(nblk), dim3(LIN_BLOCK), 0, st, cur,
                         sc.state->s[0].Tr, n_src, tgt, tgt_normals, n_tgt, sc.best, prm->dist_thresh, partials,
                         nullptr, tidx(it, 1));
    }
    {
      GsProf prof(GS_PROF_SOLVE, 1.0, st);
      hipLaunchKernelGGL(gs_icp_update_kernel, dim3(1), dim3(SUM_BLOCK), 0, st, partials, nblk, sc.state, *prm, it,
                         compose16, out_T16);
    }
    cur_in = cur;
  }
  GS_LAUNCH_CHECK();
  if (tape) return icp_tape_finish(tape, sc.state, n_src, prm->numiters, st);
  return GS_OK;
}

extern "C" int gs_icp_f32(const float* src, int64_t n_src, const float* tgt, const float* tgt_normals,
                          int64_t n_tgt, const float* init16, const float* compose16,
                          const gs_icp_params* prm, float* out_T16, int64_t* out_idx, void* icp_scratch,
                          void* stream) {
  return icp_run(src, n_src, tgt, tgt_normals, n_tgt, init16, compose16, prm, out_T16, out_idx, icp_scratch, nullptr,
                 stream);
}

extern "C" int gs_icp_dc_f32(const float* src, int64_t n_src_bound, const int64_t* n_src_dev, const float* tgt,
                             const float* tgt_normals, int64_t n_tgt_bound, const int64_t* n_tgt_dev,
                             const float* init16, const float* compose16, const gs_icp_params* prm, float* out_T16,
                             int64_t* out_idx, void* icp_scratch, void* stream) {
  return icp_run(src, n_src_bound, tgt, tgt_normals, n_tgt_bound, init16, compose16, prm, out_T16, out_idx,
                 icp_scratch, nullptr, stream, n_src_dev, n_tgt_dev);
}

extern "C" int gs_icp_map_dc_f32(const float* src, int64_t n_src_bound, const int64_t* n_src_dev,
                                 const float* map_points, const float* map_normals, const int32_t* pix,
                                 int64_t n_map_bound, const int64_t* n_map_dev, int W, int ds, const float* init16,
                                 const float* compose16, const gs_icp_params* prm, float* out_T16,
                                 void* icp_scratch, void* stream) {
  GS_REQUIRE(pix && W > 0 && ds > 0, "bad target filter");
  return icp_run(src, n_src_bound, map_points, map_normals, n_map_bound, init16, compose16, prm, out_T16, nullptr,
                 icp_scratch, nullptr, stream, n_src_dev, n_map_dev, GsTargetFilter{pix, W, ds, 1});
}

static int localize_chunk(const gs_localize_seq* seqs, int B, int H, int W, int ds, const gs_icp_params* prm,
                          hipStream_t st, bool grid_cleared) {
  const int64_t n_lat = loc_lattice(H, W, ds);
  LocLayout layouts[GS_MAX_BATCH]; LocCarve c[GS_MAX_BATCH];
  for (int b = 0; b < B; ++b) {
    layouts[b] = loc_layout(n_lat, loc_rows(seqs[b].map));
    c[b] = loc_carve(seqs[b].scratch, layouts[b]);
  }
  const IcpEnginePlan plan = icp_engine_plan(gs_env(), icp_device(), B, n_lat, prm->numiters, layouts);
  LocBatch lb; GsGridBatch gb; IcpSolveView v[GS_MAX_BATCH];
  loc_bind(seqs, B, H, W, ds, prm, plan, c, lb, gb, v);
  int rc = loc_prep(seqs, lb, gb, st, grid_cleared);
  if (rc != GS_OK) return rc;
  if (prm->numiters == 0) { GS_LAUNCH_CHECK(); return GS_OK; }
  double prof_bytes = 0.0;
  if (g_gs_prof_on && (rc = loc_prof_bytes(B, c, n_lat, prm->numiters, st, &prof_bytes)) != GS_OK) return rc;
  {
    GsProf prof(GS_PROF_ICP_FUSED, prof_bytes, st, 2 * prm->numiters);
    loc_half_iterations(v, B, plan, GsCount{n_lat, nullptr}, prm, st, false);
    if (plan.persist_on) loc_persist(v, B, plan, n_lat, prm, st);
  }
  loc_finish(v, B, plan, GsCount{n_lat, nullptr}, prm, st);
  GS_LAUNCH_CHECK();
  return GS_OK;
}

static int localize_batch(const gs_localize_seq* seqs_host, int B, int H, int W, int ds, const gs_icp_params* prm,
                          void* stream, bool grid_cleared) {
  GS_REQUIRE(seqs_host && prm && B > 0 && H > 0 && W > 0 && ds > 0, "bad arguments");
  GS_REQUIRE(!icp_params_error(prm), icp_params_error(prm));
  GS_REQUIRE((int64_t)H * W < (1ll << 31), "image too large for int32 pixel ids");
  for (int b = 0; b < B; ++b) {
    const gs_localize_seq& q = seqs_host[b];
    GS_REQUIRE(q.vertex && q.depth && q.K16 && q.prev_pose16 && q.out_pose16 && q.scratch, "NULL pointer");
    GS_REQUIRE(q.map.points && q.map.normals && q.map.n_bound > 0 && q.map.n_bound < 0x7fffffffll,
               "every sequence needs a non-empty map (points + normals)");
    GS_REQUIRE(q.map.capacity <= 0 || q.map.n_bound <= q.map.capacity, "map.n_bound exceeds map.capacity");
  }
  hipStream_t st = gs_stream(stream);
  for (int c0 = 0; c0 < B; c0 += GS_MAX_BATCH) {
    const int nb = B - c0 < GS_MAX_BATCH ? B - c0 : GS_MAX_BATCH;
    const int rc = localize_chunk(seqs_host + c0, nb, H, W, ds, prm, st, grid_cleared);
    if (rc != GS_OK) return rc;
  }
  return GS_OK;
}
extern "C" int gs_localize_batch_f32(const gs_localize_seq* seqs_host, int B, int H, int W, int ds,
                                     const gs_icp_params* prm, void* stream) {
  return localize_batch(seqs_host, B, H, W, ds, prm, stream, false);
}

__global__ void __launch_bounds__(256) gs_far_stats_kernel(const int* __restrict__ far_idx, const int* __restrict__ far_n,
                                                          const float* __restrict__ d2prev, const float4* __restrict__ far_cq,
                                                          int64_t n_lat, int* __restrict__ out4) {
  const int n0 = far_n[0], n = n0 < 0 ? 0 : (n0 > (int)n_lat ? (int)n_lat : n0);
  if (blockIdx.x == 0 && threadIdx.x == 0) { out4[0] = n; out4[2] = far_n[1]; }
  int c = 0, built = 0;
  for (int i = blockIdx.x * 256 + threadIdx.x; i < n; i += gridDim.x * 256) {
    const int s = far_idx[i];
    if (s < 0 || s >= (int)n_lat) continue;
    c += (__float_as_uint(d2prev[s]) >> 31) ? 1 : 0;
    built += far_cq[s].w > 0.0f ? 1 : 0;
  }
  if (c) atomicAdd(&out4[1], c);
  if (built) atomicAdd(&out4[3], built);
}
extern "C" int gs_localize_far_stats_i64(const void* scratch, int H, int W, int ds, int64_t map_rows, int64_t* out4_host,
                                         void* stream) {
  GS_REQUIRE(scratch && out4_host && H > 0 && W > 0 && ds > 0 && map_rows > 0, "bad arguments");
  const int64_t n_lat = loc_lattice(H, W, ds);
  const LocCarve cv = loc_carve_of(scratch, H, W, ds, map_rows);
  const FarMem& fm = cv.fm; hipStream_t st = gs_stream(stream);
  int* out4 = cv.far_out4;
  GS_HIP(hipMemsetAsync(out4, 0, 16, st));
  hipLaunchKernelGGL(gs_far_stats_kernel, dim3(64), dim3(256), 0, st, fm.idx, fm.n, reinterpret_cast<const float*>(cv.sc.best),
                     fm.cq, n_lat, out4);
  int h[4] = {0, 0, 0, 0};
  GsGrid g;
  GS_HIP(hipMemcpyAsync(h, out4, 16, hipMemcpyDeviceToHost, st));
  GS_HIP(hipMemcpyAsync(&g, cv.gm.g, sizeof(g), hipMemcpyDeviceToHost, st));
  GS_HIP(hipStreamSynchronize(st));
  for (int i = 0; i < 4; ++i) out4_host[i] = h[i];
  if (gs_env().debug_grid)
    fprintf(stderr, "grid: box (%.3f %.3f %.3f)-(%.3f %.3f %.3f) c %.4f cells %d x %d x %d = %d\n", g.ox, g.oy, g.oz, g.mx,
            g.my, g.mz, g.c, g.nx, g.ny, g.nz, g.ncell);
  return GS_OK;
}

extern "C" int gs_localize_list_stats_i64(const void* scratch, int H, int W, int ds, int64_t map_rows, int64_t* out192_host,
                                          void* stream) {
  GS_REQUIRE(scratch && out192_host && H > 0 && W > 0 && ds > 0 && map_rows > 0, "bad arguments");
  const ListMem lm = loc_carve_of(scratch, H, W, ds, map_rows).lm;
  int h[3 * GL_STAT_LAUNCHES];
  hipStream_t st = gs_stream(stream);
  GS_HIP(hipMemcpyAsync(h, lm.stat, sizeof(h), hipMemcpyDeviceToHost, st));
  GS_HIP(hipStreamSynchronize(st));
  for (int i = 0; i < 3 * GL_STAT_LAUNCHES; ++i) out192_host[i] = h[i];
  return GS_OK;
}

extern "C" int gs_localize_solve_stats_i64(const void* scratch, int H, int W, int ds, int64_t map_rows, int64_t* out8_host,
                                           void* stream) {
  GS_REQUIRE(scratch && out8_host && H > 0 && W > 0 && ds > 0 && map_rows > 0, "bad arguments");
  const LocCarve cv = loc_carve_of(scratch, H, W, ds, map_rows);
  unsigned h[PS_WORDS];
  hipStream_t st = gs_stream(stream);
  GS_HIP(hipMemcpyAsync(h, cv.sc.sync, sizeof(h), hipMemcpyDeviceToHost, st));
  GS_HIP(hipStreamSynchronize(st));
  static_assert(PS_WORDS == 8, "out8");
  for (int i = 0; i < PS_WORDS; ++i) out8_host[i] = h[i];
  return GS_OK;
}

extern "C" int gs_pointfusion_step_batch_f32(const gs_step_seq* seqs_host, int B, int H, int W, int ds,
                                             const gs_icp_params* prm, float two_sigma_sq, float dist_th, float dot_th,
                                             int renorm_all, void* stream) {
  GS_REQUIRE(seqs_host && prm && B > 0 && H > 0 && W > 0 && ds > 0, "bad arguments");
  const int64_t P = (int64_t)H * W;
  const gs_step_seq& s0 = seqs_host[0];
  const int64_t dstride = B > 1 ? seqs_host[1].depth - s0.depth : P;
  for (int b = 0; b < B; ++b) {
    const gs_step_seq& q = seqs_host[b];
    GS_REQUIRE(q.depth && q.rgb && q.K16 && q.prev_pose16 && q.out_pose16 && q.vertex && q.normal && q.alpha &&
                   q.best_pix && q.new_count_out && q.loc_scratch && q.upd_scratch, "NULL pointer");
    GS_REQUIRE((q.gvertex != nullptr) == (q.gnormal != nullptr) && (q.gvertex != nullptr) == (s0.gvertex != nullptr),
               "gvertex / gnormal: both or none, the same choice for every sequence");
    GS_REQUIRE(q.out_pose16 != q.prev_pose16, "out_pose16 must not alias prev_pose16");
    GS_REQUIRE(q.vertex == s0.vertex + 3 * P * b && q.normal == s0.normal + 3 * P * b && q.alpha == s0.alpha + P * b,
               "vertex / normal / alpha of the batch must be dense");
    GS_REQUIRE(q.depth == s0.depth + dstride * b && q.K16 == s0.K16 + 16 * (int64_t)b, "depth / K16 must be equally strided");
  }
  GS_REQUIRE(dstride >= P || B == 1, "overlapping depth images");
  const bool implicit_global = s0.gvertex == nullptr;
  std::unique_ptr<gs_update_seq[]> us(new gs_update_seq[B]);
  for (int c0 = 0; c0 < B; c0 += GS_MAX_BATCH) {
    const int nb = B - c0 < GS_MAX_BATCH ? B - c0 : GS_MAX_BATCH;
    const gs_step_seq* sq = seqs_host + c0;
    gs_localize_seq ls[GS_MAX_BATCH];
    for (int b = 0; b < nb; ++b) {
      const gs_step_seq& q = sq[b];
      ls[b].vertex = q.vertex; ls[b].depth = q.depth; ls[b].K16 = q.K16; ls[b].prev_pose16 = q.prev_pose16;
      ls[b].map = q.map; ls[b].out_pose16 = q.out_pose16; ls[b].scratch = q.loc_scratch;
      gs_update_seq& u = us[c0 + b];
      u.map = q.map; u.vertex = q.vertex; u.normal = q.normal; u.depth = q.depth; u.rgb = q.rgb;
      u.alpha = q.alpha; u.pose16 = q.out_pose16; u.K16 = q.K16; u.gvertex = q.gvertex;
      u.gnormal = q.gnormal; u.best_pix = q.best_pix; u.new_count_out = q.new_count_out;
      u.scratch = q.upd_scratch;
    }
    GsClearJob job;
    job.n = nb;
    for (int b = 0; b < nb; ++b) {
      GS_REQUIRE(ls[b].map.points && ls[b].map.n_bound > 0, "every sequence needs a non-empty map");
      const LocCarve cv = loc_carve_of(ls[b].scratch, H, W, ds, loc_rows(ls[b].map));
      job.ptr[b] = reinterpret_cast<char*>(cv.gm.g);
      if (b == 0) job.bytes = gs_knn_grid_clear_bytes(cv.gm, gs_knn_grid_cells_cap(loc_lattice(H, W, ds)));
    }
    GsPixelTables tabs{};
    tabs.n = implicit_global ? nb : 0;
    tabs.call_flag = c0 == 0 ? gs_update_map_call_flag(seqs_host[0].upd_scratch) : nullptr;
    for (int b = 0; b < tabs.n; ++b) {
      gs_update_map_tables(sq[b].upd_scratch, &tabs.any_flag[b], &tabs.key_pix[b]);
      tabs.best_pix[b] = sq[b].best_pix;
    }
    int rc = gs_frame_maps_batch_clear(sq[0].depth, dstride, P, sq[0].K16, nb, 1, H, W, two_sigma_sq, sq[0].vertex,
                                       sq[0].normal, sq[0].alpha, &job, stream, &tabs);
    if (rc != GS_OK) return rc;
    rc = localize_batch(ls, nb, H, W, ds, prm, stream, true);
    if (rc != GS_OK) return rc;
  }
  return gs_update_map_fusion_batch_impl(us.get(), B, H, W, dist_th, dot_th, renorm_all, stream, implicit_global);
}

extern "C" int64_t gs_icp_tape_bytes(int64_t n_src, int numiters) { return (int64_t)gs_icp_tape_size(n_src, numiters); }

extern "C" int gs_icp_tape_f32(const float* src, int64_t n_src, const float* tgt, const float* tgt_normals,
                               int64_t n_tgt, const float* init16, const float* compose16,
                               const gs_icp_params* prm, float* out_T16, int64_t* out_idx, void* icp_scratch,
                               void* tape, void* stream) {
  GS_REQUIRE(tape, "tape must not be NULL");
  return icp_run(src, n_src, tgt, tgt_normals, n_tgt, init16, compose16, prm, out_T16, out_idx, icp_scratch, tape,
                 stream);
}

extern "C" int gs_icp_trace_f32(const void* icp_scratch, int numiters, float* trace_out, void* stream) {
  GS_REQUIRE(icp_scratch && trace_out && numiters >= 0 && numiters <= GS_ICP_MAX_ITERS, "bad arguments");
  const GsIcpState* st = reinterpret_cast<const GsIcpState*>(icp_scratch);
  GS_HIP(hipMemcpyAsync(trace_out, st->trace, sizeof(float) * 12 * (size_t)numiters, hipMemcpyDeviceToDevice,
                        gs_stream(stream)));
  return GS_OK;
}
```

### gradslam_amd/csrc/gs_knn.h

```cpp
#pragma once
#include "gs_common.h"

GS_DEV unsigned long long knn_pack(float d, uint32_t idx) {
  return ((unsigned long long)__float_as_uint(d) << 32) | (unsigned long long)idx;
}

int gs_knn_brute_launch(const float* src_in, const float* Tapply, float* src_out, int64_t n_src,
                        const float* tgt, int64_t n_tgt, unsigned long long* best, hipStream_t st);

constexpr int GS_GRID_MAXCELL = 1 << 22;
constexpr int GS_GRID_RINGS = 3;
constexpr int GS_GRID_TILE = 1024;

struct GsGrid {
  float ox, oy, oz;
  float mx, my, mz;
  float c, inv_c;
  int nx, ny, nz, ncell;
};

struct GsTargetFilter {
  const int32_t* pix;
  int W, ds;
  int listed;
};
GS_DEV bool gs_is_target(const GsTargetFilter& f, int64_t n) {
  if (!f.pix) return true;
  const int32_t p = f.pix[n];
  return p >= 0 && ((p / f.W) % f.ds == 0) && ((p % f.W) % f.ds == 0);
}

struct GridMem {
  GsGrid* g;
  unsigned* bbox;
  int* unres_count;
  int* cell_count;
  int* cell_start;
  int* tile_sums;
  float4* sorted;
  float4* sorted_n;
  float4* tlist;
  int* unres_list;
};

static inline GridMem grid_carve(void* scratch, int64_t n_src, int64_t n_tgt) {
  char* p = reinterpret_cast<char*>(scratch);
  GridMem m;
  m.g = reinterpret_cast<GsGrid*>(p); p += 128;
  m.bbox = reinterpret_cast<unsigned*>(p); p += 128;
  m.unres_count = reinterpret_cast<int*>(p); p += 256;
  m.tile_sums = reinterpret_cast<int*>(p); p += gs_align(4 * (size_t)(GS_GRID_MAXCELL / GS_GRID_TILE + 2));
  m.cell_count = reinterpret_cast<int*>(p); p += gs_align(4 * (size_t)(GS_GRID_MAXCELL + 1));
  m.cell_start = reinterpret_cast<int*>(p); p += gs_align(4 * (size_t)(GS_GRID_MAXCELL + 1));
  m.sorted = reinterpret_cast<float4*>(p); p += gs_align(16 * (size_t)(n_tgt > 0 ? n_tgt : 1));
  m.sorted_n = reinterpret_cast<float4*>(p); p += gs_align(16 * (size_t)(n_tgt > 0 ? n_tgt : 1));
  m.tlist = reinterpret_cast<float4*>(p); p += gs_align(16 * (size_t)(n_tgt > 0 ? n_tgt : 1));
  m.unres_list = reinterpret_cast<int*>(p);
  (void)n_src;
  return m;
}

size_t gs_knn_grid_scratch_bytes(int64_t n_src, int64_t n_tgt);

struct GsGridSeq {
  const float* tgt;
  GsCount n_tgt;
  int32_t* pix;
  const float* pose16;
  const float* K16;
  const float* nrm;
  GridMem m;
};
struct GsGridBatch {
  int B, H, W, ds;
  int listed;
  int cells_cap;
  GsGridSeq s[GS_MAX_BATCH];
};
int gs_knn_grid_cells_cap(int64_t n_src);
size_t gs_knn_grid_clear_bytes(const GridMem& m, int cells_cap);
int gs_knn_grid_build_batch(const GsGridBatch& gb, hipStream_t st, bool bbox_done = false);

int gs_knn_grid_build(const float* tgt, GsCount n_tgt, int64_t n_src, void* grid_scratch, hipStream_t st,
                      GsTargetFilter filter = GsTargetFilter{nullptr, 1, 1, 0}, const float* nrm = nullptr);
int gs_knn_grid_query(const float* src_in, const float* Tapply, float* src_out, int64_t n_src,
                      const float* tgt, int64_t n_tgt, unsigned long long* best, void* grid_scratch,
                      hipStream_t st);
static inline bool gs_knn_use_grid(int64_t n_src, int64_t n_tgt) { return n_tgt >= 2048 && n_src >= 256; }

GS_DEV int grid_axis(float v, float o, float inv_c, int n) {
  const float f = (v - o) * inv_c;
  return f >= 0.0f ? (f < (float)n ? (int)f : n - 1) : 0;
}
GS_DEV int grid_cell(const GsGrid& g, float x, float y, float z) {
  const int ix = grid_axis(x, g.ox, g.inv_c, g.nx);
  const int iy = grid_axis(y, g.oy, g.inv_c, g.ny);
  const int iz = grid_axis(z, g.oz, g.inv_c, g.nz);
  return (iz * g.ny + iy) * g.nx + ix;
}

constexpr int GQ_G = 8;
constexpr int GL_RING_NF = 2;

GS_DEV unsigned long long grid_key(float qx, float qy, float qz, const float4 p) {
  const float dx = qx - p.x, dy = qy - p.y, dz = qz - p.z;
  float d = dx * dx;
  d = gs_fma(dy, dy, d);
  d = gs_fma(dz, dz, d);
  return d == d ? knn_pack(d, (uint32_t)__float_as_int(p.w)) : ~0ull;
}

template <int G>
GS_DEV unsigned long long grid_group_min(unsigned long long key) {
#pragma unroll
  for (int d = G / 2; d > 0; d >>= 1) {
    const unsigned long long o = __shfl_xor(key, d, G);
    key = o < key ? o : key;
  }
  return key;
}

struct GsQueryCell {
  float px, py, pz;
  int cx, cy, cz;
};
GS_DEV GsQueryCell grid_query_cell(const GsGrid& g, float qx, float qy, float qz) {
  GsQueryCell c;
  c.px = qx < g.ox ? g.ox : (qx > g.mx ? g.mx : qx);
  c.py = qy < g.oy ? g.oy : (qy > g.my ? g.my : qy);
  c.pz = qz < g.oz ? g.oz : (qz > g.mz ? g.mz : qz);
  c.cx = grid_axis(c.px, g.ox, g.inv_c, g.nx); c.cy = grid_axis(c.py, g.oy, g.inv_c, g.ny);
  c.cz = grid_axis(c.pz, g.oz, g.inv_c, g.nz);
  return c;
}

template <int G>
GS_DEV unsigned long long grid_search_stage0(const GsGrid& g, const int* __restrict__ cell_start,
                                             const float4* __restrict__ sorted, float qx, float qy, float qz, int lane,
                                             bool* resolved, int* win, const float rball = __builtin_inff()) {
  const GsQueryCell qc = grid_query_cell(g, qx, qy, qz);
  const float px = qc.px, py = qc.py, pz = qc.pz;
  const int cx = qc.cx, cy = qc.cy, cz = qc.cz;
  unsigned long long key = ~0ull;
  int bt = -1;
  const float fx = (px - g.ox) * g.inv_c - (float)cx, fy = (py - g.oy) * g.inv_c - (float)cy,
              fz = (pz - g.oz) * g.inv_c - (float)cz;
  const int x0 = (fx < 0.5f) ? cx - 1 : cx, y0 = (fy < 0.5f) ? cy - 1 : cy, z0 = (fz < 0.5f) ? cz - 1 : cz;
  const float BIG = 3.0e38f;
  const float ax = fminf(x0 >= 1 ? fx + (float)(cx - x0) : BIG, x0 + 2 < g.nx ? (float)(x0 + 2 - cx) - fx : BIG);
  const float ay = fminf(y0 >= 1 ? fy + (float)(cy - y0) : BIG, y0 + 2 < g.ny ? (float)(y0 + 2 - cy) - fy : BIG);
  const float az = fminf(z0 >= 1 ? fz + (float)(cz - z0) : BIG, z0 + 2 < g.nz ? (float)(z0 + 2 - cz) - fz : BIG);
  const float amin = fminf(ax, fminf(ay, az));
  const float rc = rball * g.inv_c * 1.0001f + 0.002f;
  const bool prune = rc < amin - 0.001f;
  bool ulx = true, uhx = true, uly = true, uhy = true, ulz = true, uhz = true;
  if (prune) {
    const float tx = fx + (float)(cx - x0), ty = fy + (float)(cy - y0), tz = fz + (float)(cz - z0);
    ulx = tx - rc < 1.0f; uhx = tx + rc >= 1.0f;
    uly = ty - rc < 1.0f; uhy = ty + rc >= 1.0f;
    ulz = tz - rc < 1.0f; uhz = tz + rc >= 1.0f;
  }
  int sb0 = 0, sb1 = 0, sb2 = 0, sb3 = 0, e1 = 0, e2 = 0, e3 = 0, total = 0;
  {
    const int xa = (x0 >= 0 && ulx) ? x0 : x0 + 1, xb = (x0 + 1 < g.nx && uhx) ? x0 + 1 : x0;
// ... 623 lines not shown
```

### gradslam_amd/csrc/gs_knn.hip

```cpp
#include "gs_knn.h"

#include <stdlib.h>

#include "gs_assoc_dev.h"
#include "gs_env.h"
#include "gs_knn_bbox.h"

constexpr int KNN_BLOCK = 256;
constexpr int KNN_TCHUNK = 512;

template <bool LISTED, int KNN_SPT>
__global__ void __launch_bounds__(KNN_BLOCK) gs_knn1_kernel(
    const float* __restrict__ src_in, const float* __restrict__ Tapply, float* __restrict__ src_out,
    int64_t n_src, const float* __restrict__ tgt, int64_t n_tgt, unsigned long long* __restrict__ best,
    const int* __restrict__ list, const int* __restrict__ count) {
  constexpr int KNN_STILE = KNN_BLOCK * KNN_SPT;
  __shared__ float4 tl[KNN_TCHUNK];
  const int64_t n_q = LISTED ? (int64_t)(*count) : n_src;
  if (LISTED && n_q == 0) return;
  const int64_t j0 = (int64_t)blockIdx.y * KNN_TCHUNK;
  const int cnt = (int)((n_tgt - j0) < KNN_TCHUNK ? (n_tgt - j0) : KNN_TCHUNK);
  if (cnt <= 0) return;
  for (int i = threadIdx.x; i < cnt; i += KNN_BLOCK) {
    const float* t = tgt + 3 * (j0 + i);
// ... 165 lines not shown
                                                            int cells_cap, const float4* __restrict__ tlist) {
  grid_count_body(tgt, gs_count(n_tgt_c), flt, bbox, gp, cell_count, tile_sums, cells_cap, tlist, blockIdx.x, gridDim.x);
}

GS_DEV void grid_scan_body(const int* __restrict__ cell_count, const GsGrid* __restrict__ gp,
                           const int* __restrict__ tile_sums, int* __restrict__ cell_start, const unsigned blk) {
  __shared__ int smem[256 / GS_WAVE + 1];
  const int n = gp->ncell + 1;
  if ((int)(blk * GS_GRID_TILE) >= n) return;
  int pre = 0;
  for (int t = threadIdx.x; t < (int)blk; t += 256) pre += tile_sums[t];
  int tile_prefix;
  (void)gs_block_excl_scan<256>(pre, smem, &tile_prefix);
  const int base = blk * GS_GRID_TILE + threadIdx.x * 4;
  int v[4], c = 0;
#pragma unroll
  for (int i = 0; i < 4; ++i) {
    v[i] = (base + i < n) ? cell_count[base + i] : 0;
    c += v[i];
  }
  int total;
  int run = tile_prefix + gs_block_excl_scan<256>(c, smem, &total);
#pragma unroll
  for (int i = 0; i < 4; ++i) {
    if (base + i < n) cell_start[base + i] = run;
    run += v[i];
  }
}
__global__ void __launch_bounds__(256) gs_grid_scan_kernel(const int* __restrict__ cell_count,
                                                           const GsGrid* __restrict__ gp,
                                                           const int* __restrict__ tile_sums,
                                                           int* __restrict__ cell_start) {
  grid_scan_body(cell_count, gp, tile_sums, cell_start, blockIdx.x);
}

GS_DEV void grid_scatter_body(const float* __restrict__ tgt, const int64_t n_tgt, const GsTargetFilter flt,
                              const GsGrid* __restrict__ gp, const int* __restrict__ cell_start,
                              int* __restrict__ cell_count, float4* __restrict__ sorted,
                              const float4* __restrict__ tlist, const unsigned* __restrict__ bbox,
                              const float* __restrict__ nrm, float4* __restrict__ sorted_n, const unsigned blk,
                              const unsigned nblk) {
  if (flt.listed) {
    const int64_t n_list = (int64_t)bbox[6];
    if ((int64_t)blk * 256 >= n_list) return;
    const GsGrid g = *gp;
    for (int64_t i = (int64_t)blk * 256 + threadIdx.x; i < n_list; i += (int64_t)nblk * 256) {
      const float4 t = tlist[i];
      const int cid = grid_cell(g, t.x, t.y, t.z);
      const int slot = cell_start[cid] + atomicSub(&cell_count[cid], 1) - 1;
      sorted[slot] = t;
      if (nrm) {
        const int64_t r = (int64_t)__float_as_int(t.w);
        sorted_n[slot] = make_float4(nrm[3 * r], nrm[3 * r + 1], nrm[3 * r + 2], 0.0f);
      }
    }
    return;
  }
  const int64_t i = (int64_t)blk * 256 + threadIdx.x;
  if (i >= n_tgt) return;
  const GsGrid g = *gp;
  const float x = tgt[3 * i], y = tgt[3 * i + 1], z = tgt[3 * i + 2];
  const int cid = grid_cell(g, x, y, z);
  const int slot = cell_start[cid] + atomicSub(&cell_count[cid], 1) - 1;
  sorted[slot] = make_float4(x, y, z, __int_as_float((int)i));
  if (nrm) sorted_n[slot] = make_float4(nrm[3 * i], nrm[3 * i + 1], nrm[3 * i + 2], 0.0f);
}
__global__ void __launch_bounds__(256) gs_grid_scatter_kernel(const float* __restrict__ tgt, GsCount n_tgt_c,
                                                              const GsTargetFilter flt,
                                                              const GsGrid* __restrict__ gp,
                                                              const int* __restrict__ cell_start,
                                                              int* __restrict__ cell_count,
                                                              float4* __restrict__ sorted,
                                                              const float4* __restrict__ tlist,
                                                              const unsigned* __restrict__ bbox,
                                                              const float* __restrict__ nrm,
                                                              float4* __restrict__ sorted_n) {
  grid_scatter_body(tgt, gs_count(n_tgt_c), flt, gp, cell_start, cell_count, sorted, tlist, bbox, nrm, sorted_n, blockIdx.x,
                    gridDim.x);
}

__global__ void __launch_bounds__(GB_BLOCK) gs_gridb_bbox_kernel(const GsGridBatch gb, float u_hi, float v_hi) {
  gridb_bbox_block(gb, blockIdx.x, u_hi, v_hi);
}
__global__ void __launch_bounds__(256) gs_gridb_count_kernel(const GsGridBatch gb) {
  const GsGridSeq& q = gb.s[blockIdx.x % gb.B];
  grid_count_body(q.tgt, gs_count(q.n_tgt), GsTargetFilter{q.pix, gb.W, gb.ds, gb.listed}, q.m.bbox, q.m.g, q.m.cell_count,
                  q.m.tile_sums, gb.cells_cap, q.m.tlist, blockIdx.x / gb.B, gridDim.x / gb.B);
}
__global__ void __launch_bounds__(256) gs_gridb_scan_kernel(const GsGridBatch gb) {
  const GsGridSeq& q = gb.s[blockIdx.x % gb.B];
  grid_scan_body(q.m.cell_count, q.m.g, q.m.tile_sums, q.m.cell_start, blockIdx.x / gb.B);
}
__global__ void __launch_bounds__(256) gs_gridb_scatter_kernel(const GsGridBatch gb) {
  const GsGridSeq& q = gb.s[blockIdx.x % gb.B];
  grid_scatter_body(q.tgt, gs_count(q.n_tgt), GsTargetFilter{q.pix, gb.W, gb.ds, gb.listed}, q.m.g, q.m.cell_start, q.m.cell_count,
                    q.m.sorted, q.m.tlist, q.m.bbox, q.nrm, q.m.sorted_n, blockIdx.x / gb.B, gridDim.x / gb.B);
}

static int grid_cells_cap(int64_t n_src, int64_t n_tgt_exact) {
  int64_t want = 48 * n_src;
  if (16 * n_tgt_exact > want) want = 16 * n_tgt_exact;
  int cells_cap = 1 << 20;
  while (cells_cap < GS_GRID_MAXCELL && cells_cap < want) cells_cap <<= 1;
  return cells_cap;
}
int gs_knn_grid_cells_cap(int64_t n_src) { return grid_cells_cap(n_src, 0); }
size_t gs_knn_grid_clear_bytes(const GridMem& m, int cells_cap) {
  return gs_align((size_t)(reinterpret_cast<char*>(m.cell_count) - reinterpret_cast<char*>(m.g)) +
                  4 * (size_t)(cells_cap + 1));
}

int gs_knn_grid_build_batch(const GsGridBatch& gb, hipStream_t st, bool bbox_done) {
  int64_t n_max = 1;
  for (int b = 0; b < gb.B; ++b) n_max = gb.s[b].n_tgt.host > n_max ? gb.s[b].n_tgt.host : n_max;
  const unsigned B = (unsigned)gb.B;
  const float u_hi = (float)((double)gb.W - 0.999), v_hi = (float)((double)gb.H - 0.999);
  if (!bbox_done)
    hipLaunchKernelGGL(gs_gridb_bbox_kernel, dim3(gs_knn_gridb_bbox_blocks(gb)), dim3(GB_BLOCK), 0, st, gb, u_hi, v_hi);
  const bool listed = gb.listed != 0;
  const int64_t slots = (int64_t)gs_ceil_div(gb.H, gb.ds) * gs_ceil_div(gb.W, gb.ds);
  unsigned nb_pts = (unsigned)gs_ceil_div(n_max, 256);
  if (listed && gb.H > 0 && (unsigned)gs_ceil_div(3 * slots, 256) < nb_pts) nb_pts = (unsigned)gs_ceil_div(3 * slots, 256);
  hipLaunchKernelGGL(gs_gridb_count_kernel, dim3(B * nb_pts), dim3(256), 0, st, gb);
  const unsigned ntile = (unsigned)gs_ceil_div(gb.cells_cap + 1, GS_GRID_TILE);
  hipLaunchKernelGGL(gs_gridb_scan_kernel, dim3(B * ntile), dim3(256), 0, st, gb);
  hipLaunchKernelGGL(gs_gridb_scatter_kernel, dim3(B * nb_pts), dim3(256), 0, st, gb);
  hipError_t e = hipGetLastError();
  if (e != hipSuccess) { gs_set_error("gs_knn_grid_build_batch: %s", hipGetErrorString(e)); return GS_ERR_HIP; }
  return GS_OK;
}

int gs_knn_grid_build(const float* tgt, GsCount n_tgt_c, int64_t n_src, void* grid_scratch, hipStream_t st,
                      GsTargetFilter flt, const float* nrm) {
  const int64_t n_tgt = n_tgt_c.host;
  GridMem m = grid_carve(grid_scratch, n_src, n_tgt);
  const int cells_cap = grid_cells_cap(n_src, n_tgt_c.dev ? 0 : n_tgt);
  GsProf prof(GS_PROF_COMPACT, 28.0 * (double)n_tgt + 8.0 * (double)cells_cap, st);
  const size_t clear = gs_knn_grid_clear_bytes(m, cells_cap);
  hipError_t e = hipMemsetAsync(m.g, 0, clear, st);
  if (e != hipSuccess) { gs_set_error("gs_knn_grid_build: %s", hipGetErrorString(e)); return GS_ERR_HIP; }
  hipLaunchKernelGGL(gs_grid_bbox_kernel, dim3((unsigned)gs_ceil_div(n_tgt > 0 ? n_tgt : 1, GB_BLOCK * GB_ITEMS)),
                     dim3(GB_BLOCK), 0, st, tgt, n_tgt_c, flt, m.bbox, m.unres_count, m.tlist);
  hipLaunchKernelGGL(gs_grid_count_kernel, dim3((unsigned)gs_ceil_div(n_tgt > 0 ? n_tgt : 1, 256)), dim3(256), 0, st,
                     tgt, n_tgt_c, flt, m.bbox, m.g, m.cell_count, m.tile_sums, cells_cap, m.tlist);
  const unsigned ntile = (unsigned)gs_ceil_div(cells_cap + 1, GS_GRID_TILE);
  hipLaunchKernelGGL(gs_grid_scan_kernel, dim3(ntile), dim3(256), 0, st, m.cell_count, m.g, m.tile_sums,
                     m.cell_start);
  hipLaunchKernelGGL(gs_grid_scatter_kernel, dim3((unsigned)gs_ceil_div(n_tgt, 256)), dim3(256), 0, st, tgt,
                     n_tgt_c, flt, m.g, m.cell_start, m.cell_count, m.sorted, m.tlist, m.bbox, nrm, m.sorted_n);
  return GS_OK;
}

constexpr int GQ_BLOCK = 256;

__global__ void __launch_bounds__(GQ_BLOCK) gs_grid_query_kernel(
    const float* __restrict__ src_in, const float* __restrict__ Tapply, float* __restrict__ src_out,
    int64_t n_src, const GsGrid* __restrict__ gp, const int* __restrict__ cell_start,
    const float4* __restrict__ sorted, unsigned long long* __restrict__ best, int* __restrict__ unres_count,
    int* __restrict__ unres_next, int* __restrict__ unres_list) {
  const int lane = threadIdx.x & (GQ_G - 1);
  const int64_t s = ((int64_t)blockIdx.x * GQ_BLOCK + threadIdx.x) / GQ_G;
  if (blockIdx.x == 0 && threadIdx.x == 0) *unres_next = 0;
  if (s >= n_src) return;
  const GsGrid g = *gp;
  float qx = src_in[3 * s], qy = src_in[3 * s + 1], qz = src_in[3 * s + 2];
  if (Tapply) {
    float T[12];
#pragma unroll
    for (int i = 0; i < 12; ++i) T[i] = Tapply[i];
    float t0, t1, t2;
    gs_rigid_fma(T, qx, qy, qz, t0, t1, t2);
    qx = t0; qy = t1; qz = t2;
  }
  if (src_out && lane == 0) {
    src_out[3 * s] = qx;
    src_out[3 * s + 1] = qy;
    src_out[3 * s + 2] = qz;
  }
  bool done;
  const unsigned long long key = grid_search_group(g, cell_start, sorted, qx, qy, qz, lane, &done);
  if (lane == 0) {
    if (done) {
      best[s] = key;
    } else {
      best[s] = ~0ull;
      unres_list[atomicAdd(unres_count, 1)] = (int)s;
    }
  }
}

int gs_knn_grid_query(const float* src_in, const float* Tapply, float* src_out, int64_t n_src,
                      const float* tgt, int64_t n_tgt, unsigned long long* best, void* grid_scratch,
                      hipStream_t st) {
  static unsigned seq = 0;
  GridMem m = grid_carve(grid_scratch, n_src, n_tgt);
  int* cnt = m.unres_count + (seq & 1);
  int* nxt = m.unres_count + ((seq + 1) & 1);
  ++seq;
  GsProf prof(GS_PROF_KNN, (double)n_src * (double)n_tgt, st);
  hipLaunchKernelGGL(gs_grid_query_kernel, dim3((unsigned)gs_ceil_div(n_src * GQ_G, GQ_BLOCK)), dim3(GQ_BLOCK), 0, st,
                     src_in, Tapply, src_out, n_src, m.g, m.cell_start, m.sorted, best, cnt, nxt, m.unres_list);
  unsigned gx = (unsigned)gs_ceil_div(n_src, KNN_BLOCK * 4);
  gx = gx > 4 ? 4 : gx;
  dim3 grid(gx, (unsigned)gs_ceil_div(n_tgt, KNN_TCHUNK));
  hipLaunchKernelGGL((gs_knn1_kernel<true, 4>), grid, dim3(KNN_BLOCK), 0, st, src_in, Tapply, nullptr, n_src, tgt,
                     n_tgt, best, m.unres_list, cnt);
  return GS_OK;
}

// ... 57 lines not shown
```

### gradslam_amd/slam/_fastpath.py

```python
import os

import torch

from .. import _C, ops
from ..structures.pointclouds import _ATTRS
from .fusionutils import RENORMALIZE_UNMATCHED

__all__ = ["try_step"]

f32 = torch.float32
FASTPATH = os.environ.get("GRADSLAM_HIP_FASTPATH", "1") != "0"
STEP_GLOBAL_MAPS = os.environ.get("GRADSLAM_HIP_STEP_GLOBAL_MAPS", "0") == "1"


def _kwargs_key(kw):
    def norm(v):
        if torch.is_tensor(v):
            return ("tensor", id(v), int(v._version), tuple(v.shape), str(v.dtype), str(v.device))
        return v
    return tuple(sorted((k, norm(v)) for k, v in kw.items()))


def _dense_frames(t, inner):
    if t.dtype != f32 or t.stride()[2:] != inner:
        return None
    B = t.shape[0]
    sb = t.stride(0) if B > 1 else inner[0] * t.shape[2]
    if B > 1 and sb < inner[0] * t.shape[2]:
        return None
    return t.data_ptr(), sb


class StepPlan(object):
    def __init__(self, slam, B, H, W, device):
        self.B, self.H, self.W, self.P, self.device = B, H, W, H * W, device
        self.lib = _C.lib()
        self.seqs = (_C.StepSeq * B)()
        prov = slam.odomprov
        kw = prov._kwargs()
        self.kw_tensors = [v for v in kw.values() if torch.is_tensor(v)]
        self.prm = _C.IcpParams(int(prov._mode), int(kw.get("numiters", 20)), float(kw.get("damp", 1e-8)),
                                ops._thresh(kw.get("dist_thresh")), float(kw.get("lambda_max", 2.0)),
                                float(kw.get("B", 1.0)), float(kw.get("B2", 1.0)), float(kw.get("nu", 200.0)))
        self.key = (float(slam.sigma), float(slam.dist_th), float(slam.dot_th), int(slam.dsratio), _kwargs_key(kw),
                    int(prov._mode))
        self.sigma = float(slam.sigma)
        self.tss = ops.two_sigma_sq(slam.sigma)
        self.dist_th, self.dot_th, self.ds = float(slam.dist_th), float(slam.dot_th), int(slam.dsratio)
        self.caps = [-1] * B
        self.bufs = [None] * B
        self.scratch = [None] * B
        self.stream = _C.stream(device)
        self.stream_id = torch.cuda.current_stream(device).cuda_stream

    def _bind_map(self, pc, b):
        bufs = tuple(pc._buf[k][b] for k in _ATTRS)
        cap = int(bufs[0].shape[0])
        if any(t.shape[0] != cap for t in bufs):
            return False
        q = self.seqs[b]
        m = q.map
        m.points, m.normals, m.colors, m.ccounts = (t.data_ptr() for t in bufs)
        m.capacity = cap
        if cap != self.caps[b]:
            ws = _C.Workspace.get(self.device)
            loc = ws.bytes("localize%d" % b, self.lib.gs_localize_scratch_bytes(self.H, self.W, self.ds, cap))
            upd = ws.bytes("map_update%d" % b, self.lib.gs_update_map_scratch_bytes(cap, self.H, self.W))
            self.scratch[b] = (loc, upd)
            q.loc_scratch, q.upd_scratch = loc.data_ptr(), upd.data_ptr()
            self.caps[b] = cap
        self.bufs[b] = bufs
        return True

    def run(self, pc, live, prev):
        B, P, H, W = self.B, self.P, self.H, self.W
        dev = self.device
        d = _dense_frames(live._depth_image, (W, 1, 1))
        r = _dense_frames(live._rgb_image, (3 * W, 3, 1))
        K, pp = live._intrinsics, prev._poses
        if d is None or r is None or K.dtype != f32 or pp.dtype != f32 or not K.is_contiguous() or not pp.is_contiguous():
            return None
        grp = pc._dcount[0].group
        grp.poll()
        bounds = grp.bounds
        for b in range(B):
            bufs = self.bufs[b]
            if (bufs is None or any(bufs[i] is not pc._buf[k][b] for i, k in enumerate(_ATTRS)) or
                    bounds[b] + P > self.caps[b]):
                if bounds[b] + P > int(pc._buf["points"][b].shape[0]):
                    pc._reserve(b, P, pc.RESERVE_FRAMES)
                    bounds = grp.bounds
                if not self._bind_map(pc, b):
                    return None
        gm = STEP_GLOBAL_MAPS
        out = torch.empty(B * (13 if gm else 7) * P, dtype=f32, device=dev)
        poses_out = torch.empty(B * 16, dtype=f32, device=dev)
        best = torch.empty((B, P), dtype=torch.int32, device=dev)
        o = out.data_ptr()
        v0, n0, a0, po0 = o, o + 12 * P * B, o + 24 * P * B, poses_out.data_ptr()
        gv0, gn0 = o + 28 * P * B, o + 28 * P * B + 12 * P * B
        pair = getattr(grp, "_step_counts", None)
        if pair is None or pair[0].shape[0] != B or pair[0].device != dev:
            pair = grp._step_counts = [torch.zeros(B, dtype=torch.int64, device=dev) for _ in range(2)]
        cnt_new = pair[0] if pair[0].data_ptr() != grp.dev.data_ptr() else pair[1]
        d0, ds_ = d
        r0, rs_ = r
        k0, p0, c0, n_dev0, b0 = K.data_ptr(), pp.data_ptr(), cnt_new.data_ptr(), grp.dev.data_ptr(), best.data_ptr()
        seqs = self.seqs
        for b in range(B):
            q = seqs[b]
            q.depth, q.rgb = d0 + 4 * ds_ * b, r0 + 4 * rs_ * b
            q.K16, q.prev_pose16, q.out_pose16 = k0 + 64 * b, p0 + 64 * b, po0 + 64 * b
            q.vertex, q.normal, q.alpha = v0 + 12 * P * b, n0 + 12 * P * b, a0 + 4 * P * b
            q.gvertex, q.gnormal = (gv0 + 12 * P * b, gn0 + 12 * P * b) if gm else (None, None)
            q.best_pix = b0 + 4 * P * b
            q.new_count_out = c0 + 8 * b
            q.map.n_bound = bounds[b]
            q.map.n_dev = n_dev0 + 8 * b
        _C.check(self.lib.gs_pointfusion_step_batch_f32(seqs, B, H, W, self.ds, self.prm, self.tss, self.dist_th,
                                                        self.dot_th, 1 if RENORMALIZE_UNMATCHED else 0, self.stream), "gs_pointfusion_step_batch_f32")
        n3 = 3 * P * B
        live._vertex_map = out[:n3].view(B, 1, H, W, 3)
        live._normal_map = out[n3:2 * n3].view(B, 1, H, W, 3)
        live._alpha_cache = (self.sigma, out[2 * n3:2 * n3 + P * B].view(B, 1, H, W, 1))
        live._poses = poses_out.view(B, 1, 4, 4)
        if gm:
            g = 7 * P * B
            live._global_vertex_map = out[g:g + n3].view(B, 1, H, W, 3)
            live._global_normal_map = out[g + n3:g + 2 * n3].view(B, 1, H, W, 3)
        else:
            live._global_vertex_map = live._global_normal_map = None
        grp.advance(cnt_new, P)
        pc._generation += 1
        pc._padded_cache.clear()
        pc.equisized = True if B == 1 else None
        return pc, live._poses


def try_step(slam, pointclouds, live_frame, prev_frame):
    if not ops.DEVICE_COUNTS or not FASTPATH or prev_frame is None or slam.odom not in ("icp", "gradicp"):
        return None
    B = len(pointclouds._n_host)
    dc = pointclouds._dcount
    if B == 0 or len(dc) != B:
        return None
    g0 = dc[0].group
    if len(g0.bounds) != B or any(dc[b].group is not g0 or dc[b].index != b for b in range(B)) or min(g0.bounds) <= 0:
        return None
    if live_frame._channels_first or prev_frame._channels_first or live_frame._L != 1 or live_frame._B != B:
        return None
    if prev_frame._poses is None or live_frame._intrinsics.data_ptr() != prev_frame._intrinsics.data_ptr():
        return None
    if tuple(prev_frame._poses.shape) != (B, 1, 4, 4):
        return None
    dev = live_frame.device
    if dev.type != "cuda" or pointclouds.device != dev or prev_frame.device != dev:
        return None
    bufs = pointclouds._buf
    if any(bufs[k] is None for k in _ATTRS) or bufs["points"][0].dtype != f32 or bufs["features"][0].shape[-1] != 1:
        return None
    if torch.is_grad_enabled() and (live_frame._depth_image.requires_grad or live_frame._rgb_image.requires_grad or
                                    prev_frame._poses.requires_grad or
                                    any(t.requires_grad for k in _ATTRS for t in bufs[k])):
        return None
    from ..odometry.gradicp import GradICPOdometryProvider
    from ..odometry.icp import ICPOdometryProvider
    if type(slam.odomprov) not in (ICPOdometryProvider, GradICPOdometryProvider):
        return None
    H, W = live_frame.h, live_frame.w
    plan = getattr(slam, "_step_plan", None)
    key = (float(slam.sigma), float(slam.dist_th), float(slam.dot_th), int(slam.dsratio),
           _kwargs_key(slam.odomprov._kwargs()), int(slam.odomprov._mode))
    if (plan is None or (plan.B, plan.H, plan.W, plan.device) != (B, H, W, dev) or plan.key != key or
            plan.stream_id != torch.cuda.current_stream(dev).cuda_stream):
        plan = slam._step_plan = StepPlan(slam, B, H, W, dev)
    return plan.run(pointclouds, live_frame, prev_frame)
```

Measured before the change: 3996.

## Ride frame-map tiles inside KNN grid-build kernels and skip alpha map

Moves the frame vertex/normal map computation out of its own launch and spreads its tiles as extra 'rider' blocks across the three KNN grid build kernels (count, scan, scatter). A separate small kernel clears the per-step buffers and table flags. The alpha map is no longer written by default; fusion recomputes alpha from the vertex on the fly. The aim is to fill idle CUs during the small grid-build kernels and cut launch and memory traffic, at the cost of more complex kernels with mixed block roles and recomputed alpha.

```diff
diff --git a/gradslam_amd/csrc/build.py b/gradslam_amd/csrc/build.py
--- a/gradslam_amd/csrc/build.py
+++ b/gradslam_amd/csrc/build.py
@@ -5,7 +5,7 @@
 
 HERE = os.path.dirname(os.path.abspath(__file__))
 SOURCES = ["gs_frame.hip", "gs_assoc.hip", "gs_fuse.hip", "gs_knn.hip", "gs_icp.hip", "gs_icp_loop.hip", "gs_icp_bwd.hip", "gs_ingest.hip", "gs_render.hip", "gs_prune.hip", "gs_bilateral.hip"]
-HEADERS = ["gs_common.h", "gs_env.h", "gs_compact.h", "gs_assoc_dev.h", "gs_knn.h", "gs_knn_bbox.h", "gs_icp_math.h", "gs_icp_persist.h", "gs_icp_timeline.h", os.path.join("..", "..", "include", "gradslam_hip.h")]
+HEADERS = ["gs_common.h", "gs_env.h", "gs_compact.h", "gs_frame_maps.h", "gs_assoc_dev.h", "gs_knn.h", "gs_knn_bbox.h", "gs_icp_math.h", "gs_icp_persist.h", "gs_icp_timeline.h", os.path.join("..", "..", "include", "gradslam_hip.h")]
 LIB = os.path.join(HERE, "libgradslam_hip.so")
 FLAGS = ["--offload-arch=gfx950", "-O3", "-std=c++17", "-fPIC", "-ffp-contract=off", "-fno-fast-math", "-fno-slp-vectorize",
          "-fvisibility=hidden", "-Wall", "-Wno-unused-function"]
diff --git a/gradslam_amd/csrc/gs_common.h b/gradslam_amd/csrc/gs_common.h
--- a/gradslam_amd/csrc/gs_common.h
+++ b/gradslam_amd/csrc/gs_common.h
@@ -26,9 +26,10 @@
                               int n_frames, int frames_per_K, int H, int W, float two_sigma_sq, float* vertex,
                               float* normal, float* alpha, const GsClearJob* job, void* stream,
                               const GsPixelTables* tables = nullptr);
+int gs_clear_job_tables(const GsClearJob* job, const GsPixelTables* tables, void* stream);
 
 int gs_update_map_fusion_batch_impl(const gs_update_seq* seqs_host, int B, int H, int W, float dist_th, float dot_th,
-                                    int renorm_all, void* stream, bool tables_ready);
+                                    int renorm_all, void* stream, bool tables_ready, float two_sigma_sq);
 int32_t* gs_update_map_call_flag(void* scratch_of_first_sequence);
 void gs_update_map_tables(void* scratch, int32_t** any_flag, uint64_t** key_pix);
 
diff --git a/gradslam_amd/csrc/gs_env.h b/gradslam_amd/csrc/gs_env.h
--- a/gradslam_amd/csrc/gs_env.h
+++ b/gradslam_amd/csrc/gs_env.h
@@ -17,6 +17,7 @@
   const char* icp_persist_timeline;
   bool icp_timeline_it_set; int icp_timeline_it;
   int timeline_it(int numiters) const { return icp_timeline_it_set ? icp_timeline_it : numiters - 1; }
+  int step_riders;
   bool knn_brute;
   int knn_spt;
   bool debug_grid;
@@ -42,6 +43,8 @@
     v.icp_persist_timeline = getenv("GRADSLAM_HIP_ICP_PERSIST_TIMELINE");
     v.icp_timeline_it_set = getenv("GRADSLAM_HIP_ICP_TIMELINE_IT") != nullptr;
     v.icp_timeline_it = num("GRADSLAM_HIP_ICP_TIMELINE_IT", 0);
+    v.step_riders = num("GRADSLAM_HIP_STEP_RIDERS", 1);
+    if (v.step_riders < 0 || v.step_riders > 2) v.step_riders = 1;
     const char* knn = getenv("GRADSLAM_HIP_KNN");
     v.knn_brute = knn && strcmp(knn, "brute") == 0;
     v.knn_spt = num("GRADSLAM_HIP_KNN_SPT", 0);
diff --git a/gradslam_amd/csrc/gs_frame.hip b/gradslam_amd/csrc/gs_frame.hip
--- a/gradslam_amd/csrc/gs_frame.hip
+++ b/gradslam_amd/csrc/gs_frame.hip
@@ -2,6 +2,7 @@
 #include <string.h>
 
 #include "gs_compact.h"
+#include "gs_frame_maps.h"
 
 static thread_local char g_err[512] = "";
 
@@ -101,117 +102,42 @@
   if (threadIdx.x == 0 && count_out) count_out[0] = gs_count(base_count) + carry;
 }
 
-constexpr int FM_TW = 64;
-constexpr int FM_TH = 8;
-constexpr int FM_LW = FM_TW + 2;
-constexpr int FM_LH = FM_TH + 2;
-
-GS_DEV void fm_vertex(float d, int h, int w, const GsKinv& k, float& x, float& y, float& z) {
-  float u = (float)w, v = (float)h;
-  float ax = k.k00 * u;
-  ax = gs_fma(0.0f, v, ax);
-  ax = gs_fma(k.k02, 1.0f, ax);
-  float ay = 0.0f * u;
-  ay = gs_fma(k.k11, v, ay);
-  ay = gs_fma(k.k12, 1.0f, ay);
-  float az = 0.0f * u;
-  az = gs_fma(0.0f, v, az);
-  az = gs_fma(1.0f, 1.0f, az);
-  float validf = d > 0.0f ? 1.0f : 0.0f;
-  x = (ax * d) * validf;
-  y = (ay * d) * validf;
-  z = (az * d) * validf;
-}
-
-struct GsRow3 {
-  float x, y, z;
-};
-GS_DEV void frame_maps_body(const float* __restrict__ depth, const float* __restrict__ K16, int H, int W,
-                            float two_sigma_sq, float* __restrict__ vertex, float* __restrict__ normal,
-                            float* __restrict__ alpha, uint8_t* __restrict__ valid,
-                            uint64_t* __restrict__ key_pix = nullptr, int32_t* __restrict__ best_pix = nullptr) {
-  __shared__ float tile[FM_LH][FM_LW];
-  const int w_base = blockIdx.x * FM_TW, h_base = blockIdx.y * FM_TH;
-  for (int i = threadIdx.x; i < FM_LH * FM_LW; i += 256) {
-    int lh = i / FM_LW, lw = i - lh * FM_LW;
-    int gh = h_base + lh - 1, gw = w_base + lw - 1;
-    gh = gh < 0 ? 0 : (gh > H - 1 ? H - 1 : gh);
-    gw = gw < 0 ? 0 : (gw > W - 1 ? W - 1 : gw);
-    tile[lh][lw] = depth[(size_t)gh * W + gw];
-  }
-  __syncthreads();
-  const GsKinv k = gs_kinv(K16);
-  const int lane = threadIdx.x & 63, wave = threadIdx.x >> 6;
-  const int w = w_base + lane;
-  if (w >= W) return;
-#pragma unroll
-  for (int r = 0; r < 2; ++r) {
-    const int lh = wave * 2 + r;
-    const int h = h_base + lh;
-    if (h >= H) continue;
-    const size_t p = (size_t)h * W + w;
-    const float d = tile[lh + 1][lane + 1];
-    float vx, vy, vz;
-    fm_vertex(d, h, w, k, vx, vy, vz);
-    if (vertex) reinterpret_cast<GsRow3*>(vertex)[p] = GsRow3{vx, vy, vz};
-    if (valid) valid[p] = d > 0.0f ? 1 : 0;
-    if (alpha) alpha[p] = gs_alpha_of(vx, vy, vz, two_sigma_sq, 1e-7f);
-    if (key_pix) { key_pix[p] = ~0ull; best_pix[p] = -1; }
-    if (normal) {
-      const int w0 = (w < W - 1) ? w : W - 2;
-      const int h0 = (h < H - 1) ? h : H - 2;
-      const int lw0 = w0 - w_base + 1, lh0 = h0 - h_base + 1;
-      float a0x, a0y, a0z, a1x, a1y, a1z, b0x, b0y, b0z, b1x, b1y, b1z;
-      fm_vertex(tile[lh + 1][lw0], h, w0, k, a0x, a0y, a0z);
-      fm_vertex(tile[lh + 1][lw0 + 1], h, w0 + 1, k, a1x, a1y, a1z);
-      fm_vertex(tile[lh0][lane + 1], h0, w, k, b0x, b0y, b0z);
-      fm_vertex(tile[lh0 + 1][lane + 1], h0 + 1, w, k, b1x, b1y, b1z);
-      const float dhx = a1x - a0x, dhy = a1y - a0y, dhz = a1z - a0z;
-      const float dvx = b1x - b0x, dvy = b1y - b0y, dvz = b1z - b0z;
-      const float nx = gs_fma(dhy, dvz, -(dhz * dvy));
-      const float ny = gs_fma(dhz, dvx, -(dhx * dvz));
-      const float nz = gs_fma(dhx, dvy, -(dhy * dvx));
-      const float nrm = gs_norm3(nx, ny, nz);
-      const float den = (nrm == 0.0f) ? 1.0f : nrm;
-      const float validf = d > 0.0f ? 1.0f : 0.0f;
-      reinterpret_cast<GsRow3*>(normal)[p] = GsRow3{(nx / den) * validf, (ny / den) * validf, (nz / den) * validf};
-    }
-  }
-}
-
 __global__ void __launch_bounds__(256) gs_frame_maps_kernel(
     const float* __restrict__ depth, const float* __restrict__ K16, int H, int W, float two_sigma_sq,
     float* __restrict__ vertex, float* __restrict__ normal, float* __restrict__ alpha,
     uint8_t* __restrict__ valid) {
-  frame_maps_body(depth, K16, H, W, two_sigma_sq, vertex, normal, alpha, valid);
+  frame_maps_body(blockIdx.x, blockIdx.y, depth, K16, H, W, two_sigma_sq, vertex, normal, alpha, valid);
+}
+GS_DEV void clear_job_block(const GsClearJob& job, const size_t blk) {
+  const size_t n16 = job.bytes / 16, per = (n16 + 256 * GS_CLEAR_ITEMS - 1) / (256 * GS_CLEAR_ITEMS);
+  const size_t r = blk / per;
+  if (r >= (size_t)job.n) return;
+  float4* dst = reinterpret_cast<float4*>(job.ptr[r]);
+  const size_t base = (blk % per) * 256 * GS_CLEAR_ITEMS + threadIdx.x;
+#pragma unroll
+  for (int u = 0; u < GS_CLEAR_ITEMS; ++u) {
+    const size_t i = base + (size_t)u * 256;
+    if (i < n16) dst[i] = make_float4(0.0f, 0.0f, 0.0f, 0.0f);
+  }
+}
+GS_DEV void clear_table_flags(const GsPixelTables& tabs, const int f) {
+  tabs.any_flag[f][0] = 0;
+  tabs.any_flag[f][1] = 0;
+  if (f == 0 && tabs.call_flag) *tabs.call_flag = 0;
 }
 __global__ void __launch_bounds__(256) gs_frame_maps_batch_kernel(
     const float* __restrict__ depth, int64_t stride_seq, int64_t stride_frame, const float* __restrict__ K16,
     int frames_per_K, int H, int W, float two_sigma_sq, float* __restrict__ vertex, float* __restrict__ normal,
     float* __restrict__ alpha, const int n_frames, const GsClearJob job, const GsPixelTables tabs) {
   if ((int)blockIdx.z >= n_frames) {
-    const size_t blk = ((size_t)(blockIdx.z - n_frames) * gridDim.y + blockIdx.y) * gridDim.x + blockIdx.x;
-    const size_t n16 = job.bytes / 16, per = (n16 + 256 * GS_CLEAR_ITEMS - 1) / (256 * GS_CLEAR_ITEMS);
-    const size_t r = blk / per;
-    if (r >= (size_t)job.n) return;
-    float4* dst = reinterpret_cast<float4*>(job.ptr[r]);
-    const size_t base = (blk % per) * 256 * GS_CLEAR_ITEMS + threadIdx.x;
-#pragma unroll
-    for (int u = 0; u < GS_CLEAR_ITEMS; ++u) {
-      const size_t i = base + (size_t)u * 256;
-      if (i < n16) dst[i] = make_float4(0.0f, 0.0f, 0.0f, 0.0f);
-    }
+    clear_job_block(job, ((size_t)(blockIdx.z - n_frames) * gridDim.y + blockIdx.y) * gridDim.x + blockIdx.x);
     return;
   }
   const size_t f = blockIdx.z, P = (size_t)H * W;
   const size_t b = f / frames_per_K, l = f % frames_per_K;
   const bool tb = (int)f < tabs.n;
-  if (tb && blockIdx.x == 0 && blockIdx.y == 0 && threadIdx.x == 0) {
-    tabs.any_flag[f][0] = 0;
-    tabs.any_flag[f][1] = 0;
-    if (f == 0 && tabs.call_flag) *tabs.call_flag = 0;
-  }
-  frame_maps_body(depth + b * stride_seq + l * stride_frame, K16 + 16 * b, H, W, two_sigma_sq, vertex + 3 * f * P,
+  if (tb && blockIdx.x == 0 && blockIdx.y == 0 && threadIdx.x == 0) clear_table_flags(tabs, (int)f);
+  frame_maps_body(blockIdx.x, blockIdx.y, depth + b * stride_seq + l * stride_frame, K16 + 16 * b, H, W, two_sigma_sq, vertex + 3 * f * P,
                   normal ? normal + 3 * f * P : nullptr, alpha ? alpha + f * P : nullptr, nullptr,
                   tb ? tabs.key_pix[f] : nullptr, tb ? tabs.best_pix[f] : nullptr);
 }
@@ -261,6 +187,20 @@
   GsProf prof(GS_PROF_FRAME, bytes, gs_stream(stream));
   hipLaunchKernelGGL(gs_frame_maps_batch_kernel, grid, dim3(256), 0, gs_stream(stream), depth, depth_stride_seq,
                      depth_stride_frame, K16, frames_per_K, H, W, two_sigma_sq, vertex, normal, alpha, n_frames, *job, tabs);
+  GS_LAUNCH_CHECK();
+  return GS_OK;
+}
+
+__global__ void __launch_bounds__(256) gs_clear_job_kernel(const GsClearJob job, const GsPixelTables tabs) {
+  if (blockIdx.x == 0 && (int)threadIdx.x < tabs.n) clear_table_flags(tabs, (int)threadIdx.x);
+  clear_job_block(job, blockIdx.x);
+}
+int gs_clear_job_tables(const GsClearJob* job, const GsPixelTables* tables, void* stream) {
+  GS_REQUIRE(job && job->n > 0 && job->n <= GS_MAX_BATCH && job->bytes > 0 && job->bytes % 16 == 0, "bad clear job");
+  GS_REQUIRE(tables && tables->n >= 0 && tables->n <= GS_MAX_BATCH, "bad pixel tables");
+  const int64_t per = gs_ceil_div((int64_t)(job->bytes / 16), 256 * GS_CLEAR_ITEMS);
+  GsProf prof(GS_PROF_COMPACT, (double)job->n * (double)job->bytes, gs_stream(stream));
+  hipLaunchKernelGGL(gs_clear_job_kernel, dim3((unsigned)(per * job->n)), dim3(256), 0, gs_stream(stream), *job, *tables);
   GS_LAUNCH_CHECK();
   return GS_OK;
 }
diff --git a/gradslam_amd/csrc/gs_frame_maps.h b/gradslam_amd/csrc/gs_frame_maps.h
--- /dev/null
+++ b/gradslam_amd/csrc/gs_frame_maps.h
@@ -0,0 +1,107 @@
+#pragma once
+#include "gs_common.h"
+
+constexpr int FM_TW = 64;
+constexpr int FM_TH = 8;
+constexpr int FM_LW = FM_TW + 2;
+constexpr int FM_LH = FM_TH + 2;
+
+GS_DEV void fm_vertex(float d, int h, int w, const GsKinv& k, float& x, float& y, float& z) {
+  float u = (float)w, v = (float)h;
+  float ax = k.k00 * u;
+  ax = gs_fma(0.0f, v, ax);
+  ax = gs_fma(k.k02, 1.0f, ax);
+  float ay = 0.0f * u;
+  ay = gs_fma(k.k11, v, ay);
+  ay = gs_fma(k.k12, 1.0f, ay);
+  float az = 0.0f * u;
+  az = gs_fma(0.0f, v, az);
+  az = gs_fma(1.0f, 1.0f, az);
+  float validf = d > 0.0f ? 1.0f : 0.0f;
+  x = (ax * d) * validf;
+  y = (ay * d) * validf;
+  z = (az * d) * validf;
+}
+
+struct GsRow3 {
+  float x, y, z;
+};
+GS_DEV void frame_maps_body(const int tx, const int ty, const float* __restrict__ depth, const float* __restrict__ K16,
+                            int H, int W, float two_sigma_sq, float* __restrict__ vertex, float* __restrict__ normal,
+                            float* __restrict__ alpha, uint8_t* __restrict__ valid,
+                            uint64_t* __restrict__ key_pix = nullptr, int32_t* __restrict__ best_pix = nullptr) {
+  __shared__ float tile[FM_LH][FM_LW];
+  const int w_base = tx * FM_TW, h_base = ty * FM_TH;
+  for (int i = threadIdx.x; i < FM_LH * FM_LW; i += 256) {
+    int lh = i / FM_LW, lw = i - lh * FM_LW;
+    int gh = h_base + lh - 1, gw = w_base + lw - 1;
+    gh = gh < 0 ? 0 : (gh > H - 1 ? H - 1 : gh);
+    gw = gw < 0 ? 0 : (gw > W - 1 ? W - 1 : gw);
+    tile[lh][lw] = depth[(size_t)gh * W + gw];
+  }
+  __syncthreads();
+  const GsKinv k = gs_kinv(K16);
+  const int lane = threadIdx.x & 63, wave = threadIdx.x >> 6;
+  const int w = w_base + lane;
+  if (w >= W) return;
+#pragma unroll
+  for (int r = 0; r < 2; ++r) {
+    const int lh = wave * 2 + r;
+    const int h = h_base + lh;
+    if (h >= H) continue;
+    const size_t p = (size_t)h * W + w;
+    const float d = tile[lh + 1][lane + 1];
+    float vx, vy, vz;
+    fm_vertex(d, h, w, k, vx, vy, vz);
+    if (vertex) reinterpret_cast<GsRow3*>(vertex)[p] = GsRow3{vx, vy, vz};
+    if (valid) valid[p] = d > 0.0f ? 1 : 0;
+    if (alpha) alpha[p] = gs_alpha_of(vx, vy, vz, two_sigma_sq, 1e-7f);
+    if (key_pix) { key_pix[p] = ~0ull; best_pix[p] = -1; }
+    if (normal) {
+      const int w0 = (w < W - 1) ? w : W - 2;
+      const int h0 = (h < H - 1) ? h : H - 2;
+      const int lw0 = w0 - w_base + 1, lh0 = h0 - h_base + 1;
+      float a0x, a0y, a0z, a1x, a1y, a1z, b0x, b0y, b0z, b1x, b1y, b1z;
+      fm_vertex(tile[lh + 1][lw0], h, w0, k, a0x, a0y, a0z);
+      fm_vertex(tile[lh + 1][lw0 + 1], h, w0 + 1, k, a1x, a1y, a1z);
+      fm_vertex(tile[lh0][lane + 1], h0, w, k, b0x, b0y, b0z);
+      fm_vertex(tile[lh0 + 1][lane + 1], h0 + 1, w, k, b1x, b1y, b1z);
+      const float dhx = a1x - a0x, dhy = a1y - a0y, dhz = a1z - a0z;
+      const float dvx = b1x - b0x, dvy = b1y - b0y, dvz = b1z - b0z;
+      const float nx = gs_fma(dhy, dvz, -(dhz * dvy));
+      const float ny = gs_fma(dhz, dvx, -(dhx * dvz));
+      const float nz = gs_fma(dhx, dvy, -(dhy * dvx));
+      const float nrm = gs_norm3(nx, ny, nz);
+      const float den = (nrm == 0.0f) ? 1.0f : nrm;
+      const float validf = d > 0.0f ? 1.0f : 0.0f;
+      reinterpret_cast<GsRow3*>(normal)[p] = GsRow3{(nx / den) * validf, (ny / den) * validf, (nz / den) * validf};
+    }
+  }
+}
+
+struct GsFrameRider {
+  const float* depth; int64_t stride_seq, stride_frame;
+  const float* K16; int frames_per_K;
+  int H, W; float two_sigma_sq;
+  float *vertex, *normal, *alpha;
+  int n_frames;
+  GsPixelTables tabs;
+  unsigned begin, end;
+  int first;
+};
+static inline unsigned gs_frame_rider_tiles(const GsFrameRider& r) {
+  return (unsigned)(gs_ceil_div(r.W, FM_TW) * gs_ceil_div(r.H, FM_TH) * r.n_frames);
+}
+GS_DEV void frame_rider_block(const GsFrameRider& r, const unsigned idx) {
+  if (idx >= r.end - r.begin) return;
+  const unsigned t = r.begin + idx;
+  const unsigned ntx = (unsigned)((r.W + FM_TW - 1) / FM_TW), nty = (unsigned)((r.H + FM_TH - 1) / FM_TH);
+  const size_t f = t / (ntx * nty), P = (size_t)r.H * r.W;
+  const unsigned in = t % (ntx * nty);
+  const size_t b = f / r.frames_per_K, l = f % r.frames_per_K;
+  const bool tb = (int)f < r.tabs.n;
+  frame_maps_body((int)(in % ntx), (int)(in / ntx), r.depth + b * r.stride_seq + l * r.stride_frame, r.K16 + 16 * b, r.H, r.W,
+                  r.two_sigma_sq, r.vertex + 3 * f * P, r.normal ? r.normal + 3 * f * P : nullptr,
+                  r.alpha ? r.alpha + f * P : nullptr, nullptr, tb ? r.tabs.key_pix[f] : nullptr,
+                  tb ? r.tabs.best_pix[f] : nullptr);
+}
diff --git a/gradslam_amd/csrc/gs_fuse.hip b/gradslam_amd/csrc/gs_fuse.hip
--- a/gradslam_amd/csrc/gs_fuse.hip
+++ b/gradslam_amd/csrc/gs_fuse.hip
@@ -39,6 +39,10 @@
 #pragma unroll
     for (int k = 0; k < 3; ++k) fn[k] = gnormal[3 * p + k];
   }
+  __device__ float vertex_alpha_of(const int64_t p, float* fp, const float* __restrict__ alpha, float) const {
+    vertex_of(p, fp);
+    return alpha[p];
+  }
 };
 struct FrameLocalMaps {
   const float* __restrict__ vertex;
@@ -76,6 +80,16 @@
     fn[1] = gs_dot3_fma(T[4], T[5], T[6], n[0], n[1], n[2]);
     fn[2] = gs_dot3_fma(T[8], T[9], T[10], n[0], n[1], n[2]);
   }
+  __device__ float vertex_alpha_of(const int64_t p, float* fp, const float* __restrict__ alpha, const float two_sigma_sq) const {
+    float v[3];
+#pragma unroll
+    for (int k = 0; k < 3; ++k) v[k] = vertex[3 * p + k];
+    const float validf = v[2] > 0.0f ? 1.0f : 0.0f;
+    float g0, g1, g2;
+    gs_rigid_fma(T, v[0], v[1], v[2], g0, g1, g2);
+    fp[0] = g0 * validf; fp[1] = g1 * validf; fp[2] = g2 * validf;
+    return alpha ? alpha[p] : gs_alpha_of(v[0], v[1], v[2], two_sigma_sq, 1e-7f);
+  }
 };
 GS_DEV FrameLocalMaps frame_local_maps(const float* vertex, const float* normal, const float* pose16) {
   FrameLocalMaps f;
@@ -88,9 +102,8 @@
 template <bool HAVE_VERTEX = false, class Frame>
 GS_DEV void fuse_merge_row(float* __restrict__ points, float* __restrict__ normals, float* __restrict__ colors,
                            float* __restrict__ ccounts, const int64_t n, const int32_t p, const Frame& frame,
-                           const float* __restrict__ rgb, const float* __restrict__ alpha, const float cc,
+                           const float* __restrict__ rgb, const float a, const float cc,
                            const float* fv = nullptr) {
-  const float a = p >= 0 ? alpha[p] : 0.0f;
   float P[3], N[3], C[3], fp[3] = {0.0f, 0.0f, 0.0f}, fn[3] = {0.0f, 0.0f, 0.0f}, fc[3] = {0.0f, 0.0f, 0.0f};
 #pragma unroll
   for (int k = 0; k < 3; ++k) {
@@ -137,7 +150,8 @@
   if (*any_flag == 0 && renorm_all != 2) return;
   const int32_t p = pix_of[n];
   if (p < 0 && !renorm_all) return;
-  fuse_merge_row(points, normals, colors, ccounts, n, p, FrameGlobalMaps{gvertex, gnormal}, rgb, alpha, ccounts[n]);
+  fuse_merge_row(points, normals, colors, ccounts, n, p, FrameGlobalMaps{gvertex, gnormal}, rgb, p >= 0 ? alpha[p] : 0.0f,
+                 ccounts[n]);
 }
 
 struct PredNewPixel {
@@ -157,16 +171,18 @@
   Frame frame;
   const float* rgb;
   const float* alpha;
+  float two_sigma_sq = 0.0f;
   __device__ void operator()(int64_t p, int64_t pos) const {
     const int64_t r = gs_count(n_map) + pos;
     float v[3], nn[3] = {0.0f, 0.0f, 0.0f}, c[3] = {0.0f, 0.0f, 0.0f};
-    frame.vertex_of(p, v);
+    float a = 0.0f;
+    if (ccounts) a = frame.vertex_alpha_of(p, v, alpha, two_sigma_sq);
+    else frame.vertex_of(p, v);
     if (normals) frame.normal_of(p, nn);
     if (colors) {
 #pragma unroll
       for (int k = 0; k < 3; ++k) c[k] = rgb[3 * p + k];
     }
-    const float a = ccounts ? alpha[p] : 0.0f;
 #pragma unroll
     for (int k = 0; k < 3; ++k) points[3 * r + k] = v[k];
     if (normals) {
@@ -396,6 +412,7 @@
   int B, H, W, renorm_all;
   int64_t P, ntiles;
   float u_hi, v_hi, dist_th, dot_th;
+  float two_sigma_sq;
   int32_t* call_flag;
   int zero_call_flag;
   MuSeq s[GS_MAX_BATCH];
@@ -500,12 +517,12 @@
 GS_DEV void mu_merge_row(const MuBatch& mb, const MuSeq& q, const int64_t n, const Frame& frame) {
   int32_t p = q.pix[n];
   const float cc = q.ccounts[n];
-  float fp[3] = {0.0f, 0.0f, 0.0f};
+  float fp[3] = {0.0f, 0.0f, 0.0f}, a = 0.0f;
   if (p >= 0) {
     const uint64_t kp = q.key_pix[p];
     bool win = (uint32_t)(kp >> 32) == gs_assoc_key_hi(cc);
     if (win) {
-      frame.vertex_of((int64_t)p, fp);
+      a = frame.vertex_alpha_of((int64_t)p, fp, q.alpha, mb.two_sigma_sq);
       const int32_t bp = q.best_pix[p];
       win = (uint32_t)kp == gs_assoc_key_lo_v(q.points, fp, n) && (bp == -1 || bp == (int32_t)n);
       if (win && bp == -1) q.best_pix[p] = (int32_t)n;
@@ -513,7 +530,7 @@
     if (!win) p = -1;
   }
   if (p < 0 && !mb.renorm_all) return;
-  fuse_merge_row<true>(q.points, q.normals, q.colors, q.ccounts, n, p, frame, q.rgb, q.alpha, cc, fp);
+  fuse_merge_row<true>(q.points, q.normals, q.colors, q.ccounts, n, p, frame, q.rgb, p >= 0 ? a : 0.0f, cc, fp);
 }
 
 GS_DEV void mu_merge_body(const MuBatch& mb, const unsigned bid) {
@@ -574,7 +591,7 @@
     }
   } else {
     const EmitAppendT<FrameLocalMaps> emit{q.points, q.normals, q.colors, q.ccounts, q.n_map,
-                                           frame_local_maps(q.vertex, q.normal, q.pose16), q.rgb, q.alpha};
+                                           frame_local_maps(q.vertex, q.normal, q.pose16), q.rgb, q.alpha, mb.two_sigma_sq};
     for (int r = threadIdx.x; r < tile_new; r += GS_CP_BLOCK) {
       const int64_t pos = (int64_t)tile_prefix + r;
       if (n_map + pos < q.capacity) emit(tile_base + loc_s[r], pos);
@@ -601,9 +618,10 @@
 }
 
 static int update_chunk(const gs_update_seq* seqs, int B, int H, int W, float dist_th, float dot_th, int renorm_all,
-                        hipStream_t st, int phase, int32_t* call_flag, bool first_chunk, bool tables_ready) {
+                        hipStream_t st, int phase, int32_t* call_flag, bool first_chunk, bool tables_ready,
+                        float two_sigma_sq) {
   MuBatch mb;
-  mb.B = B; mb.H = H; mb.W = W; mb.renorm_all = renorm_all;
+  mb.B = B; mb.H = H; mb.W = W; mb.renorm_all = renorm_all; mb.two_sigma_sq = two_sigma_sq;
   mb.call_flag = call_flag; mb.zero_call_flag = first_chunk ? 1 : 0;
   mb.P = (int64_t)H * W;
   mb.ntiles = gs_cp_tiles(mb.P);
@@ -654,7 +672,7 @@
 }
 
 int gs_update_map_fusion_batch_impl(const gs_update_seq* seqs_host, int B, int H, int W, float dist_th, float dot_th,
-                                    int renorm_all, void* stream, bool tables_ready) {
+                                    int renorm_all, void* stream, bool tables_ready, float two_sigma_sq) {
   GS_REQUIRE(seqs_host && B > 0 && H > 0 && W > 0, "bad arguments");
   GS_REQUIRE((int64_t)H * W < (1ll << 31), "too large for int32 indices");
   for (int b = 0; b < B; ++b) {
@@ -662,8 +680,10 @@
     GS_REQUIRE(u.map.n_bound >= 0 && u.map.n_bound < 0x7fffffff, "bad map size");
     GS_REQUIRE(u.map.capacity >= u.map.n_bound + (int64_t)H * W, "capacity must cover n_bound + H*W rows");
     GS_REQUIRE(u.map.points && u.map.normals && u.map.colors && u.map.ccounts && u.vertex && u.normal && u.depth && u.rgb &&
-                   u.alpha && u.pose16 && u.K16 && u.best_pix && u.new_count_out && u.scratch,
+                   u.pose16 && u.K16 && u.best_pix && u.new_count_out && u.scratch,
                "NULL pointer");
+    GS_REQUIRE(u.alpha || (tables_ready && !u.gvertex && two_sigma_sq > 0.0f), "alpha may be NULL only with implicit global maps");
+    GS_REQUIRE((u.alpha != nullptr) == (seqs_host[0].alpha != nullptr), "alpha: every sequence or none");
     GS_REQUIRE((u.gvertex && u.gnormal) || (tables_ready && !u.gvertex && !u.gnormal), "gvertex / gnormal: both or none");
     GS_REQUIRE(u.new_count_out != u.map.n_dev, "new_count_out must not alias the map's device count");
   }
@@ -673,7 +693,7 @@
     for (int c0 = 0; c0 < B; c0 += GS_MAX_BATCH) {
       const int nb = B - c0 < GS_MAX_BATCH ? B - c0 : GS_MAX_BATCH;
       const int rc = update_chunk(seqs_host + c0, nb, H, W, dist_th, dot_th, renorm_all, st, phase, call_flag, c0 == 0,
-                                  tables_ready);
+                                  tables_ready, two_sigma_sq);
       if (rc != GS_OK) return rc;
     }
   }
@@ -682,7 +702,7 @@
 
 extern "C" int gs_update_map_fusion_batch_f32(const gs_update_seq* seqs_host, int B, int H, int W, float dist_th,
                                               float dot_th, int renorm_all, void* stream) {
-  return gs_update_map_fusion_batch_impl(seqs_host, B, H, W, dist_th, dot_th, renorm_all, stream, false);
+  return gs_update_map_fusion_batch_impl(seqs_host, B, H, W, dist_th, dot_th, renorm_all, stream, false, 0.0f);
 }
 
 extern "C" int gs_update_map_fusion_dc_f32(float* points, float* normals, float* colors, float* ccounts,
diff --git a/gradslam_amd/csrc/gs_icp_loop.hip b/gradslam_amd/csrc/gs_icp_loop.hip
--- a/gradslam_amd/csrc/gs_icp_loop.hip
+++ b/gradslam_amd/csrc/gs_icp_loop.hip
@@ -1039,6 +1039,7 @@
   int* lstat;
   float4* wl_cq;
   unsigned* sync;
+  const float* K16;
 };
 struct LocBatch {
   int B, W, ds, Wl;
@@ -1047,6 +1048,7 @@
   float damp;
   int numiters;
   int count_valid;
+  int vertex_from_depth;
   LocSeq s[GS_MAX_BATCH];
 };
 constexpr int LP_CLEAR_ITEMS = 8;
@@ -1060,11 +1062,18 @@
     if (e < lb.n_lat) {
       const int64_t p = (e / lb.Wl) * lb.ds * (int64_t)lb.W + (e % lb.Wl) * lb.ds;
       float g0 = __builtin_nanf(""), g1 = g0, g2 = g0;
-      if (q.depth[p] > 0.0f) {
+      const float d = q.depth[p];
+      if (d > 0.0f) {
         float T[12];
 #pragma unroll
         for (int i = 0; i < 12; ++i) T[i] = q.pose16[i];
-        gs_rigid_fma(T, q.vertex[3 * p], q.vertex[3 * p + 1], q.vertex[3 * p + 2], g0, g1, g2);
+        float v0, v1, v2;
+        if (lb.vertex_from_depth) {
+          fm_vertex(d, (int)(e / lb.Wl) * lb.ds, (int)(e % lb.Wl) * lb.ds, gs_kinv(q.K16), v0, v1, v2);
+        } else {
+          v0 = q.vertex[3 * p]; v1 = q.vertex[3 * p + 1]; v2 = q.vertex[3 * p + 2];
+        }
+        gs_rigid_fma(T, v0, v1, v2, g0, g1, g2);
         valid = 1;
       }
       q.lattice[3 * e] = g0; q.lattice[3 * e + 1] = g1; q.lattice[3 * e + 2] = g2;
@@ -1309,7 +1318,7 @@
     if (!plan.binned_normals) c[b].gm.sorted_n = nullptr;
     lb.s[b] = LocSeq{q.vertex, q.depth, q.prev_pose16, c[b].lattice, c[b].sc.state, q.out_pose16,
                      reinterpret_cast<char*>(c[b].gm.g), c[b].n_valid, c[b].fm.n, c[b].lm.stat,
-                     plan.wide_on ? c[b].fm.cq : nullptr, c[b].sc.sync};
+                     plan.wide_on ? c[b].fm.cq : nullptr, c[b].sc.sync, q.K16};
     gb.s[b] = GsGridSeq{q.map.points, GsCount{q.map.n_bound, q.map.n_dev}, nullptr, q.prev_pose16, q.K16,
                         plan.binned_normals ? q.map.normals : nullptr, c[b].gm};
     v[b] = IcpSolveView{c[b].lattice, q.map.points, q.map.normals, GsCount{q.map.n_bound, q.map.n_dev}, c[b].sc, c[b].gm,
@@ -1321,10 +1330,12 @@
                         q.prev_pose16, q.out_pose16, plan.persist_on ? c[b].sc.sync : nullptr};
   }
   lb.count_valid = g_gs_prof_on ? 1 : 0;
+  lb.vertex_from_depth = 0;
   lb.clear_bytes = gs_knn_grid_clear_bytes(c[0].gm, gb.cells_cap);
 }
 
-static int loc_prep(const gs_localize_seq* seqs, const LocBatch& lb, const GsGridBatch& gb, hipStream_t st, bool grid_cleared) {
+static int loc_prep(const gs_localize_seq* seqs, const LocBatch& lb, const GsGridBatch& gb, hipStream_t st, bool grid_cleared,
+                    const GsFrameRider* rider) {
   const int B = lb.B;
   if (g_gs_prof_on)
     for (int b = 0; b < B; ++b) GS_HIP(hipMemsetAsync(lb.s[b].n_valid, 0, 8, st));
@@ -1332,12 +1343,15 @@
   const unsigned nb_clear = (unsigned)gs_ceil_div((int64_t)(lb.clear_bytes / 16), 256 * LP_CLEAR_ITEMS);
   double bytes = 0.0;
   for (int b = 0; b < B; ++b) bytes += 28.0 * lb.n_lat + 12.0 * seqs[b].map.n_bound + 16.0 * gb.cells_cap;
+  if (rider)
+    bytes += (double)rider->H * rider->W * ((double)rider->n_frames * (16.0 + (rider->normal ? 12 : 0) + (rider->alpha ? 4 : 0)) +
+                                            12.0 * rider->tabs.n);
   GsProf prof(GS_PROF_COMPACT, bytes, st, grid_cleared ? 4 : 5);
   if (grid_cleared) {
     const float u_hi = (float)((double)gb.W - 0.999), v_hi = (float)((double)gb.H - 0.999);
     hipLaunchKernelGGL(gs_loc_prep_bbox_kernel, dim3((unsigned)B * nb_lat + gs_knn_gridb_bbox_blocks(gb)), dim3(256), 0, st,
                        lb, gb, nb_lat, u_hi, v_hi);
-    return gs_knn_grid_build_batch(gb, st, true);
+    return gs_knn_grid_build_batch(gb, st, true, rider);
   }
   hipLaunchKernelGGL(gs_loc_prep_kernel, dim3((unsigned)B * (nb_lat + nb_clear)), dim3(256), 0, st, lb, nb_lat);
   return gs_knn_grid_build_batch(gb, st);
@@ -1564,7 +1578,7 @@
 }
 
 static int localize_chunk(const gs_localize_seq* seqs, int B, int H, int W, int ds, const gs_icp_params* prm,
-                          hipStream_t st, bool grid_cleared) {
+                          hipStream_t st, bool grid_cleared, const GsFrameRider* rider) {
   const int64_t n_lat = loc_lattice(H, W, ds);
   LocLayout layouts[GS_MAX_BATCH]; LocCarve c[GS_MAX_BATCH];
   for (int b = 0; b < B; ++b) {
@@ -1574,7 +1588,8 @@
   const IcpEnginePlan plan = icp_engine_plan(gs_env(), icp_device(), B, n_lat, prm->numiters, layouts);
   LocBatch lb; GsGridBatch gb; IcpSolveView v[GS_MAX_BATCH];
   loc_bind(seqs, B, H, W, ds, prm, plan, c, lb, gb, v);
-  int rc = loc_prep(seqs, lb, gb, st, grid_cleared);
+  lb.vertex_from_depth = rider ? 1 : 0;
+  int rc = loc_prep(seqs, lb, gb, st, grid_cleared, rider);
   if (rc != GS_OK) return rc;
   if (prm->numiters == 0) { GS_LAUNCH_CHECK(); return GS_OK; }
   double prof_bytes = 0.0;
@@ -1590,10 +1605,11 @@
 }
 
 static int localize_batch(const gs_localize_seq* seqs_host, int B, int H, int W, int ds, const gs_icp_params* prm,
-                          void* stream, bool grid_cleared) {
+                          void* stream, bool grid_cleared, const GsFrameRider* rider = nullptr) {
   GS_REQUIRE(seqs_host && prm && B > 0 && H > 0 && W > 0 && ds > 0, "bad arguments");
   GS_REQUIRE(!icp_params_error(prm), icp_params_error(prm));
   GS_REQUIRE((int64_t)H * W < (1ll << 31), "image too large for int32 pixel ids");
+  GS_REQUIRE(!rider || (grid_cleared && B <= GS_MAX_BATCH && rider->n_frames == B), "a rider covers one cleared chunk");
   for (int b = 0; b < B; ++b) {
     const gs_localize_seq& q = seqs_host[b];
     GS_REQUIRE(q.vertex && q.depth && q.K16 && q.prev_pose16 && q.out_pose16 && q.scratch, "NULL pointer");
@@ -1604,7 +1620,7 @@
   hipStream_t st = gs_stream(stream);
   for (int c0 = 0; c0 < B; c0 += GS_MAX_BATCH) {
     const int nb = B - c0 < GS_MAX_BATCH ? B - c0 : GS_MAX_BATCH;
-    const int rc = localize_chunk(seqs_host + c0, nb, H, W, ds, prm, st, grid_cleared);
+    const int rc = localize_chunk(seqs_host + c0, nb, H, W, ds, prm, st, grid_cleared, rider);
     if (rc != GS_OK) return rc;
   }
   return GS_OK;
@@ -1685,12 +1701,14 @@
   const int64_t dstride = B > 1 ? seqs_host[1].depth - s0.depth : P;
   for (int b = 0; b < B; ++b) {
     const gs_step_seq& q = seqs_host[b];
-    GS_REQUIRE(q.depth && q.rgb && q.K16 && q.prev_pose16 && q.out_pose16 && q.vertex && q.normal && q.alpha &&
+    GS_REQUIRE(q.depth && q.rgb && q.K16 && q.prev_pose16 && q.out_pose16 && q.vertex && q.normal &&
                    q.best_pix && q.new_count_out && q.loc_scratch && q.upd_scratch, "NULL pointer");
+    GS_REQUIRE((q.alpha != nullptr) == (s0.alpha != nullptr) && (q.alpha || !q.gvertex),
+               "alpha: every sequence or none, and NULL only with gvertex = gnormal = NULL");
     GS_REQUIRE((q.gvertex != nullptr) == (q.gnormal != nullptr) && (q.gvertex != nullptr) == (s0.gvertex != nullptr),
                "gvertex / gnormal: both or none, the same choice for every sequence");
     GS_REQUIRE(q.out_pose16 != q.prev_pose16, "out_pose16 must not alias prev_pose16");
-    GS_REQUIRE(q.vertex == s0.vertex + 3 * P * b && q.normal == s0.normal + 3 * P * b && q.alpha == s0.alpha + P * b,
+    GS_REQUIRE(q.vertex == s0.vertex + 3 * P * b && q.normal == s0.normal + 3 * P * b && (!q.alpha || q.alpha == s0.alpha + P * b),
                "vertex / normal / alpha of the batch must be dense");
     GS_REQUIRE(q.depth == s0.depth + dstride * b && q.K16 == s0.K16 + 16 * (int64_t)b, "depth / K16 must be equally strided");
   }
@@ -1726,13 +1744,24 @@
       gs_update_map_tables(sq[b].upd_scratch, &tabs.any_flag[b], &tabs.key_pix[b]);
       tabs.best_pix[b] = sq[b].best_pix;
     }
-    int rc = gs_frame_maps_batch_clear(sq[0].depth, dstride, P, sq[0].K16, nb, 1, H, W, two_sigma_sq, sq[0].vertex,
-                                       sq[0].normal, sq[0].alpha, &job, stream, &tabs);
+    int rc;
+    if (gs_env().step_riders) {
+      GS_REQUIRE(H >= 2 && W >= 2, "image must be at least 2x2");
+      GsFrameRider rider{sq[0].depth, dstride, P, sq[0].K16, 1, H, W, two_sigma_sq, sq[0].vertex, sq[0].normal, sq[0].alpha,
+                         nb, tabs, 0u, 0u, 0};
+      GS_REQUIRE((int64_t)gs_frame_rider_tiles(rider) < (1ll << 30), "too many frame-map tiles for one chunk");
+      rc = gs_clear_job_tables(&job, &tabs, stream);
+      if (rc != GS_OK) return rc;
+      rc = localize_batch(ls, nb, H, W, ds, prm, stream, true, &rider);
+    } else {
+      rc = gs_frame_maps_batch_clear(sq[0].depth, dstride, P, sq[0].K16, nb, 1, H, W, two_sigma_sq, sq[0].vertex,
+                                     sq[0].normal, sq[0].alpha, &job, stream, &tabs);
+      if (rc != GS_OK) return rc;
+      rc = localize_batch(ls, nb, H, W, ds, prm, stream, true);
+    }
     if (rc != GS_OK) return rc;
-    rc = localize_batch(ls, nb, H, W, ds, prm, stream, true);
-    if (rc != GS_OK) return rc;
-  }
-  return gs_update_map_fusion_batch_impl(us.get(), B, H, W, dist_th, dot_th, renorm_all, stream, implicit_global);
+  }
+  return gs_update_map_fusion_batch_impl(us.get(), B, H, W, dist_th, dot_th, renorm_all, stream, implicit_global, two_sigma_sq);
 }
 
 extern "C" int64_t gs_icp_tape_bytes(int64_t n_src, int numiters) { return (int64_t)gs_icp_tape_size(n_src, numiters); }
diff --git a/gradslam_amd/csrc/gs_knn.h b/gradslam_amd/csrc/gs_knn.h
--- a/gradslam_amd/csrc/gs_knn.h
+++ b/gradslam_amd/csrc/gs_knn.h
@@ -1,5 +1,6 @@
 #pragma once
 #include "gs_common.h"
+#include "gs_frame_maps.h"
 
 GS_DEV unsigned long long knn_pack(float d, uint32_t idx) {
   return ((unsigned long long)__float_as_uint(d) << 32) | (unsigned long long)idx;
@@ -79,7 +80,7 @@
 };
 int gs_knn_grid_cells_cap(int64_t n_src);
 size_t gs_knn_grid_clear_bytes(const GridMem& m, int cells_cap);
-int gs_knn_grid_build_batch(const GsGridBatch& gb, hipStream_t st, bool bbox_done = false);
+int gs_knn_grid_build_batch(const GsGridBatch& gb, hipStream_t st, bool bbox_done = false, const GsFrameRider* rider = nullptr);
 
 int gs_knn_grid_build(const float* tgt, GsCount n_tgt, int64_t n_src, void* grid_scratch, hipStream_t st,
                       GsTargetFilter filter = GsTargetFilter{nullptr, 1, 1, 0}, const float* nrm = nullptr);
diff --git a/gradslam_amd/csrc/gs_knn.hip b/gradslam_amd/csrc/gs_knn.hip
--- a/gradslam_amd/csrc/gs_knn.hip
+++ b/gradslam_amd/csrc/gs_knn.hip
@@ -271,19 +271,34 @@
 __global__ void __launch_bounds__(GB_BLOCK) gs_gridb_bbox_kernel(const GsGridBatch gb, float u_hi, float v_hi) {
   gridb_bbox_block(gb, blockIdx.x, u_hi, v_hi);
 }
-__global__ void __launch_bounds__(256) gs_gridb_count_kernel(const GsGridBatch gb) {
-  const GsGridSeq& q = gb.s[blockIdx.x % gb.B];
+GS_DEV bool grid_rider_role(const GsFrameRider& fr, const unsigned own, unsigned* ob) {
+  const unsigned nr = fr.end - fr.begin;
+  if (fr.first) {
+    *ob = blockIdx.x < nr ? blockIdx.x : blockIdx.x - nr;
+    return blockIdx.x < nr;
+  }
+  *ob = blockIdx.x < own ? blockIdx.x : blockIdx.x - own;
+  return blockIdx.x >= own;
+}
+__global__ void __launch_bounds__(256) gs_gridb_count_kernel(const GsGridBatch gb, const GsFrameRider fr, const unsigned own) {
+  unsigned ob;
+  if (grid_rider_role(fr, own, &ob)) { frame_rider_block(fr, ob); return; }
+  const GsGridSeq& q = gb.s[ob % gb.B];
   grid_count_body(q.tgt, gs_count(q.n_tgt), GsTargetFilter{q.pix, gb.W, gb.ds, gb.listed}, q.m.bbox, q.m.g, q.m.cell_count,
-                  q.m.tile_sums, gb.cells_cap, q.m.tlist, blockIdx.x / gb.B, gridDim.x / gb.B);
-}
-__global__ void __launch_bounds__(256) gs_gridb_scan_kernel(const GsGridBatch gb) {
-  const GsGridSeq& q = gb.s[blockIdx.x % gb.B];
-  grid_scan_body(q.m.cell_count, q.m.g, q.m.tile_sums, q.m.cell_start, blockIdx.x / gb.B);
-}
-__global__ void __launch_bounds__(256) gs_gridb_scatter_kernel(const GsGridBatch gb) {
-  const GsGridSeq& q = gb.s[blockIdx.x % gb.B];
+                  q.m.tile_sums, gb.cells_cap, q.m.tlist, ob / gb.B, own / gb.B);
+}
+__global__ void __launch_bounds__(256) gs_gridb_scan_kernel(const GsGridBatch gb, const GsFrameRider fr, const unsigned own) {
+  unsigned ob;
+  if (grid_rider_role(fr, own, &ob)) { frame_rider_block(fr, ob); return; }
+  const GsGridSeq& q = gb.s[ob % gb.B];
+  grid_scan_body(q.m.cell_count, q.m.g, q.m.tile_sums, q.m.cell_start, ob / gb.B);
+}
+__global__ void __launch_bounds__(256) gs_gridb_scatter_kernel(const GsGridBatch gb, const GsFrameRider fr, const unsigned own) {
+  unsigned ob;
+  if (grid_rider_role(fr, own, &ob)) { frame_rider_block(fr, ob); return; }
+  const GsGridSeq& q = gb.s[ob % gb.B];
   grid_scatter_body(q.tgt, gs_count(q.n_tgt), GsTargetFilter{q.pix, gb.W, gb.ds, gb.listed}, q.m.g, q.m.cell_start, q.m.cell_count,
-                    q.m.sorted, q.m.tlist, q.m.bbox, q.nrm, q.m.sorted_n, blockIdx.x / gb.B, gridDim.x / gb.B);
+                    q.m.sorted, q.m.tlist, q.m.bbox, q.nrm, q.m.sorted_n, ob / gb.B, own / gb.B);
 }
 
 static int grid_cells_cap(int64_t n_src, int64_t n_tgt_exact) {
@@ -299,7 +314,15 @@
                   4 * (size_t)(cells_cap + 1));
 }
 
-int gs_knn_grid_build_batch(const GsGridBatch& gb, hipStream_t st, bool bbox_done) {
+static void grid_rider_deal(const unsigned tiles, unsigned cut[4]) {
+  const unsigned w0 = 37, w1 = 22;
+  cut[0] = 0;
+  cut[1] = (unsigned)((uint64_t)tiles * w0 / 100);
+  cut[2] = (unsigned)((uint64_t)tiles * (w0 + w1) / 100);
+  cut[3] = tiles;
+}
+
+int gs_knn_grid_build_batch(const GsGridBatch& gb, hipStream_t st, bool bbox_done, const GsFrameRider* rider) {
   int64_t n_max = 1;
   for (int b = 0; b < gb.B; ++b) n_max = gb.s[b].n_tgt.host > n_max ? gb.s[b].n_tgt.host : n_max;
   const unsigned B = (unsigned)gb.B;
@@ -310,10 +333,16 @@
   const int64_t slots = (int64_t)gs_ceil_div(gb.H, gb.ds) * gs_ceil_div(gb.W, gb.ds);
   unsigned nb_pts = (unsigned)gs_ceil_div(n_max, 256);
   if (listed && gb.H > 0 && (unsigned)gs_ceil_div(3 * slots, 256) < nb_pts) nb_pts = (unsigned)gs_ceil_div(3 * slots, 256);
-  hipLaunchKernelGGL(gs_gridb_count_kernel, dim3(B * nb_pts), dim3(256), 0, st, gb);
   const unsigned ntile = (unsigned)gs_ceil_div(gb.cells_cap + 1, GS_GRID_TILE);
-  hipLaunchKernelGGL(gs_gridb_scan_kernel, dim3(B * ntile), dim3(256), 0, st, gb);
-  hipLaunchKernelGGL(gs_gridb_scatter_kernel, dim3(B * nb_pts), dim3(256), 0, st, gb);
+  GsFrameRider fr[3] = {};
+  unsigned cut[4] = {0, 0, 0, 0};
+  if (rider) {
+    grid_rider_deal(gs_frame_rider_tiles(*rider), cut);
+    for (int i = 0; i < 3; ++i) { fr[i] = *rider; fr[i].begin = cut[i]; fr[i].end = cut[i + 1]; fr[i].first = gs_env().step_riders != 2; }
+  }
+  hipLaunchKernelGGL(gs_gridb_count_kernel, dim3(B * nb_pts + (cut[1] - cut[0])), dim3(256), 0, st, gb, fr[0], B * nb_pts);
+  hipLaunchKernelGGL(gs_gridb_scan_kernel, dim3(B * ntile + (cut[2] - cut[1])), dim3(256), 0, st, gb, fr[1], B * ntile);
+  hipLaunchKernelGGL(gs_gridb_scatter_kernel, dim3(B * nb_pts + (cut[3] - cut[2])), dim3(256), 0, st, gb, fr[2], B * nb_pts);
   hipError_t e = hipGetLastError();
   if (e != hipSuccess) { gs_set_error("gs_knn_grid_build_batch: %s", hipGetErrorString(e)); return GS_ERR_HIP; }
   return GS_OK;
diff --git a/gradslam_amd/slam/_fastpath.py b/gradslam_amd/slam/_fastpath.py
--- a/gradslam_amd/slam/_fastpath.py
+++ b/gradslam_amd/slam/_fastpath.py
@@ -11,6 +11,7 @@
 f32 = torch.float32
 FASTPATH = os.environ.get("GRADSLAM_HIP_FASTPATH", "1") != "0"
 STEP_GLOBAL_MAPS = os.environ.get("GRADSLAM_HIP_STEP_GLOBAL_MAPS", "0") == "1"
+STEP_ALPHA_MAP = os.environ.get("GRADSLAM_HIP_STEP_ALPHA_MAP", "0") == "1"
 
 
 def _kwargs_key(kw):
@@ -93,7 +94,8 @@
                 if not self._bind_map(pc, b):
                     return None
         gm = STEP_GLOBAL_MAPS
-        out = torch.empty(B * (13 if gm else 7) * P, dtype=f32, device=dev)
+        am = gm or STEP_ALPHA_MAP
+        out = torch.empty(B * (13 if gm else (7 if am else 6)) * P, dtype=f32, device=dev)
         poses_out = torch.empty(B * 16, dtype=f32, device=dev)
         best = torch.empty((B, P), dtype=torch.int32, device=dev)
         o = out.data_ptr()
@@ -111,7 +113,7 @@
             q = seqs[b]
             q.depth, q.rgb = d0 + 4 * ds_ * b, r0 + 4 * rs_ * b
             q.K16, q.prev_pose16, q.out_pose16 = k0 + 64 * b, p0 + 64 * b, po0 + 64 * b
-            q.vertex, q.normal, q.alpha = v0 + 12 * P * b, n0 + 12 * P * b, a0 + 4 * P * b
+            q.vertex, q.normal, q.alpha = v0 + 12 * P * b, n0 + 12 * P * b, (a0 + 4 * P * b) if am else None
             q.gvertex, q.gnormal = (gv0 + 12 * P * b, gn0 + 12 * P * b) if gm else (None, None)
             q.best_pix = b0 + 4 * P * b
             q.new_count_out = c0 + 8 * b
@@ -122,7 +124,7 @@
         n3 = 3 * P * B
         live._vertex_map = out[:n3].view(B, 1, H, W, 3)
         live._normal_map = out[n3:2 * n3].view(B, 1, H, W, 3)
-        live._alpha_cache = (self.sigma, out[2 * n3:2 * n3 + P * B].view(B, 1, H, W, 1))
+        live._alpha_cache = (self.sigma, out[2 * n3:2 * n3 + P * B].view(B, 1, H, W, 1)) if am else None
         live._poses = poses_out.view(B, 1, 4, 4)
         if gm:
             g = 7 * P * B
```

Result: no change. 4021 (median of 6 runs) (+0.6%).
